# facebookresearch/vggsfm

Hardware: NVIDIA H100
Metric: BA iterations/sec (higher is better)
Workload: dtype f64

## Files before the change

### vggsfm_b200/csrc/ba_schur.cu

```cuda
#include <stddef.h>
#include <algorithm>
#include <vector>
#include "common.cuh"
#include "dev_probes.h"
#include "syrk_work.h"

namespace vgg {

BandDev g_band_dev = {nullptr, nullptr, nullptr, 0};

__device__ __forceinline__ void ar_add(double* local, double* mc, double v) {
  if (mc) asm volatile("multimem.red.relaxed.sys.global.add.f64 [%0], %1;" ::"l"(mc), "d"(v) : "memory");
  else atomicAdd(local, v);
}
__device__ __forceinline__ void ar_put(double* local, double* mc, double v) {
  if (mc) asm volatile("multimem.red.relaxed.sys.global.add.f64 [%0], %1;" ::"l"(mc), "d"(v) : "memory");
  else *local = v;
}

__global__ void jacobi_scale_points_kernel(int N, const double* __restrict__ H_pp, double* __restrict__ sc_p, int enable) {
  const int n = blockIdx.x * blockDim.x + threadIdx.x;
  if (n >= N) return;
  const double* h = H_pp + (size_t)n * 6;
  sc_p[n * 3 + 0] = enable ? 1.0 / (1.0 + sqrt(h[0])) : 1.0;
  sc_p[n * 3 + 1] = enable ? 1.0 / (1.0 + sqrt(h[3])) : 1.0;
  sc_p[n * 3 + 2] = enable ? 1.0 / (1.0 + sqrt(h[5])) : 1.0;
}

__global__ void jacobi_scale_cams_kernel(int D, const double* __restrict__ hdiag, double* __restrict__ sc_c, int enable) {
  const int i = blockIdx.x * blockDim.x + threadIdx.x;
  if (i >= D) return;
  sc_c[i] = enable ? 1.0 / (1.0 + sqrt(hdiag[i])) : 1.0;
}

__global__ void point_prep_kernel(int N, const double* __restrict__ H_pp, const double* __restrict__ g_p,
                                  const double* __restrict__ sc_p, const uint8_t* __restrict__ point_const,
                                  double radius, double min_diag, double max_diag, double* __restrict__ M,
                                  double* __restrict__ q, double* __restrict__ dpp, double* __restrict__ scal) {
  const int n = blockIdx.x * blockDim.x + threadIdx.x;
  if (n >= N) return;
  double* Mo = M + (size_t)n * 9;
  if (point_const && point_const[n]) {
#pragma unroll
    for (int i = 0; i < 9; ++i) Mo[i] = 0.0;
    q[n * 3] = q[n * 3 + 1] = q[n * 3 + 2] = 0.0;
    dpp[n * 3] = dpp[n * 3 + 1] = dpp[n * 3 + 2] = 0.0;
    return;
  }
  const double* h = H_pp + (size_t)n * 6;
  const double s0 = sc_p[n * 3], s1 = sc_p[n * 3 + 1], s2 = sc_p[n * 3 + 2];
  double v00 = h[0] * s0 * s0, v01 = h[1] * s0 * s1, v02 = h[2] * s0 * s2;
  double v11 = h[3] * s1 * s1, v12 = h[4] * s1 * s2, v22 = h[5] * s2 * s2;
  const double d0 = fmin(fmax(v00, min_diag), max_diag);
  const double d1 = fmin(fmax(v11, min_diag), max_diag);
  const double d2 = fmin(fmax(v22, min_diag), max_diag);
  dpp[n * 3] = d0; dpp[n * 3 + 1] = d1; dpp[n * 3 + 2] = d2;
  v00 += d0 / radius; v11 += d1 / radius; v22 += d2 / radius;
  bool bad = !(v00 > 0.0);
  const double l00 = sqrt(v00);
  const double l10 = v01 / l00, l20 = v02 / l00;
  const double t11 = v11 - l10 * l10;
  bad = bad || !(t11 > 0.0);
  const double l11 = sqrt(t11);
  const double l21 = (v12 - l20 * l10) / l11;
  const double t22 = v22 - l20 * l20 - l21 * l21;
  bad = bad || !(t22 > 0.0);
  const double l22 = sqrt(t22);
  if (bad) {
    atomicAdd(&scal[6], 1.0);
#pragma unroll
    for (int i = 0; i < 9; ++i) Mo[i] = 0.0;
    q[n * 3] = q[n * 3 + 1] = q[n * 3 + 2] = 0.0;
    return;
  }
  const double i00 = 1.0 / l00, i11 = 1.0 / l11, i22 = 1.0 / l22;
  const double i10 = -l10 * i00 * i11;
  const double i21 = -l21 * i11 * i22;
  const double i20 = -(l20 * i00 + l21 * i10) * i22;
  const double m00 = s0 * i00, m01 = s0 * i10, m02 = s0 * i20;
  const double m11 = s1 * i11, m12 = s1 * i21;
  const double m22 = s2 * i22;
  Mo[0] = m00; Mo[1] = m01; Mo[2] = m02;
  Mo[3] = 0.0; Mo[4] = m11; Mo[5] = m12;
  Mo[6] = 0.0; Mo[7] = 0.0; Mo[8] = m22;
  const double g0 = g_p[n * 3], g1 = g_p[n * 3 + 1], g2 = g_p[n * 3 + 2];
  q[n * 3 + 0] = m00 * g0;
  q[n * 3 + 1] = m01 * g0 + m11 * g1;
  q[n * 3 + 2] = m02 * g0 + m12 * g1 + m22 * g2;
}

__global__ void assemble_hc_kernel(int S, int dc, int ns, int KR, int Dpad, const double* __restrict__ camrec,
                                   const double* __restrict__ shared_in, double* __restrict__ Sraw,
                                   double* __restrict__ rhs, double* __restrict__ hdiag, double* __restrict__ gvec,
                                   ptrdiff_t mc_off) {
  const int s = blockIdx.x;
  const int tid = threadIdx.x;
#define VGG_PUT(ptr, val) ar_put((ptr), mc_off ? (ptr) + mc_off : nullptr, (val))
  if (s < S) {
    const double* rec = camrec + (size_t)s * KR;
    const int base = s * dc;
    if (tid < dc) {
      VGG_PUT(&gvec[base + tid], rec[tid]);
      VGG_PUT(&rhs[base + tid], -rec[tid]);
    }
    if (tid < dc * dc) {
      const int i = tid / dc, j = tid % dc;
      const int a = i < j ? i : j, b = i < j ? j : i;
      const int idx = dc + a * dc - a * (a - 1) / 2 + (b - a);
      const double val = rec[idx];
      VGG_PUT(&Sraw[(size_t)(base + i) * Dpad + base + j], val);
      if (i == j) VGG_PUT(&hdiag[base + i], val);
    }
    if (tid < 6 * ns) {
      const int i = tid / ns, j = tid % ns;
      const double val = rec[dc + dc * (dc + 1) / 2 + tid];
      VGG_PUT(&Sraw[(size_t)(S * dc + j) * Dpad + base + i], val);
      VGG_PUT(&Sraw[(size_t)(base + i) * Dpad + S * dc + j], val);
    }
  } else if (ns > 0) {
    const int base = S * dc;
    if (tid < ns) {
      VGG_PUT(&gvec[base + tid], shared_in[tid]);
      VGG_PUT(&rhs[base + tid], -shared_in[tid]);
    }
    if (tid < ns * ns) {
      const int i = tid / ns, j = tid % ns;
      const int a = i < j ? i : j, b = i < j ? j : i;
      const double val = shared_in[2 + (a == 0 ? b : 2)];
      VGG_PUT(&Sraw[(size_t)(base + i) * Dpad + base + j], val);
      if (i == j) VGG_PUT(&hdiag[base + i], val);
    }
  }
#undef VGG_PUT
}

constexpr int ZB_NT = 32;
__global__ void __launch_bounds__(128) z_build_kernel(int D, int N, int Dpad, size_t pitch, const double* __restrict__ W,
                                                      const double* __restrict__ M, const double* __restrict__ q,
                                                      double* __restrict__ Zt, double* __restrict__ rhs,
                                                      ptrdiff_t mc_off, const int* __restrict__ rb_range) {
  __shared__ double sm[ZB_NT][12];
  const int row = blockIdx.x * 128 + threadIdx.x;
  const int n0 = blockIdx.y * ZB_NT;
  const int nt = min(ZB_NT, N - n0);
  if (rb_range) {
    const int kb_first = (3 * n0) >> 6, kb_last = (3 * (n0 + nt - 1) + 2) >> 6;
    if (kb_last < rb_range[2 * blockIdx.x] || kb_first >= rb_range[2 * blockIdx.x + 1]) return;
  }
  for (int e = threadIdx.x; e < nt * 12; e += 128) {
    const int t = e / 12, k = e % 12;
    sm[t][k] = k < 9 ? M[(size_t)(n0 + t) * 9 + k] : q[(size_t)(n0 + t) * 3 + (k - 9)];
  }
  __syncthreads();
  if (row >= D) return;
  double zq = 0.0;
  const double* wp = W + ((size_t)n0 * pitch + row) * 3;
#pragma unroll 4
  for (int t = 0; t < nt; ++t, wp += pitch * 3) {
    const double w0 = wp[0], w1 = wp[1], w2 = wp[2];
    const double* m = sm[t];
    const double z0 = w0 * m[0];
    const double z1 = w0 * m[1] + w1 * m[4];
    const double z2 = w0 * m[2] + w1 * m[5] + w2 * m[8];
    double* zo = Zt + (size_t)(3 * (n0 + t)) * Dpad + row;
    zo[0] = z0;
    zo[Dpad] = z1;
    zo[2 * (size_t)Dpad] = z2;
    zq += z0 * m[9] + z1 * m[10] + z2 * m[11];
  }
  if (zq != 0.0) ar_add(&rhs[row], mc_off ? &rhs[row] + mc_off : nullptr, zq);
}

constexpr int SF_BM = 128, SF_BK = 16, SF_LDS = 132, SF_STAGES = 4, SF_MMA_WARPS = 8;
constexpr int SF_THREADS = 128 + SF_MMA_WARPS * 32;
constexpr int SF_STAGE_DOUBLES = 2 * SF_BK * SF_LDS;
constexpr size_t SF_SMEM_BYTES = sizeof(double) * SF_STAGES * SF_STAGE_DOUBLES + sizeof(uint64_t) * 2 * SF_STAGES;

struct SyrkWork {
  int bi, bj, kb0, kb1;
};

__device__ __forceinline__ void dmma_m16n8k16(double (&d)[4], const double (&a)[8], const double (&b)[4]) {
  asm volatile(
      "mma.sync.aligned.m16n8k16.row.col.f64.f64.f64.f64 {%0,%1,%2,%3}, {%4,%5,%6,%7,%8,%9,%10,%11}, {%12,%13,%14,%15}, "
      "{%0,%1,%2,%3};"
      : "+d"(d[0]), "+d"(d[1]), "+d"(d[2]), "+d"(d[3])
      : "d"(a[0]), "d"(a[1]), "d"(a[2]), "d"(a[3]), "d"(a[4]), "d"(a[5]), "d"(a[6]), "d"(a[7]), "d"(b[0]), "d"(b[1]),
        "d"(b[2]), "d"(b[3]));
}

__global__ void __launch_bounds__(SF_THREADS, 1)
    syrk_f64_kernel(const SyrkWork* __restrict__ work, int nwork, int Kpad, int Dpad, const double* __restrict__ Zt,
                    double* __restrict__ Cmat, ptrdiff_t mc_off, int fill_upper, const __grid_constant__ FabricDev fd) {
  extern __shared__ __align__(16) double sf_smem[];
  uint64_t* full = reinterpret_cast<uint64_t*>(sf_smem + SF_STAGES * SF_STAGE_DOUBLES);
  uint64_t* empty = full + SF_STAGES;
  const int warp = threadIdx.x >> 5, lane = threadIdx.x & 31;
  if (threadIdx.x == 0) {
    for (int s = 0; s < SF_STAGES; ++s) {
      mbar_init(&full[s], 1);
      mbar_init(&empty[s], SF_MMA_WARPS);
    }
    mbar_fence_init();
  }
  __syncthreads();

  int stage = 0, phase = 0;
  if (warp < 4) {
    asm volatile("setmaxnreg.dec.sync.aligned.u32 40;");
    if (warp > 0) return;
    const int row = lane & (SF_BK - 1), opnd = lane / SF_BK;
    for (int w = blockIdx.x; w < nwork; w += gridDim.x) {
      const SyrkWork wk = work[w];
      const bool diag = wk.bi == wk.bj;
      const int k1 = min(Kpad, wk.kb1 * 64);
      for (int k = wk.kb0 * 64; k < k1; k += SF_BK) {
        mbar_wait(&empty[stage], phase ^ 1);
        if (lane == 0) mbar_expect_tx(&full[stage], (diag ? 1u : 2u) * SF_BK * SF_BM * (uint32_t)sizeof(double));
        __syncwarp();
        if (opnd == 0 || !diag)
          tma_load_1d(sf_smem + stage * SF_STAGE_DOUBLES + (opnd * SF_BK + row) * SF_LDS,
                      Zt + (size_t)(k + row) * Dpad + (opnd ? wk.bj : wk.bi) * SF_BM, SF_BM * sizeof(double), &full[stage]);
        if (++stage == SF_STAGES) {
          stage = 0;
          phase ^= 1;
        }
      }
    }
    return;
  }

  asm volatile("setmaxnreg.inc.sync.aligned.u32 232;");
  const int wm = (warp - 4) >> 2, wn = warp & 3;
  const int g = lane >> 2, t = lane & 3;
  for (int w = blockIdx.x; w < nwork; w += gridDim.x) {
    const SyrkWork wk = work[w];
    const bool diag = wk.bi == wk.bj;
    const int k1 = min(Kpad, wk.kb1 * 64);
    double acc[4][4][4];
#pragma unroll
    for (int mt = 0; mt < 4; ++mt)
#pragma unroll
      for (int nt = 0; nt < 4; ++nt)
#pragma unroll
        for (int h = 0; h < 4; ++h) acc[mt][nt][h] = 0.0;
    for (int k = wk.kb0 * 64; k < k1; k += SF_BK) {
      mbar_wait(&full[stage], phase);
      const double* as = sf_smem + stage * SF_STAGE_DOUBLES + t * SF_LDS + wm * 64 + g;
      const double* bs = sf_smem + stage * SF_STAGE_DOUBLES + (diag ? 0 : SF_BK * SF_LDS) + t * SF_LDS + wn * 32 + g;
      double b[4][4];
#pragma unroll
      for (int nt = 0; nt < 4; ++nt)
#pragma unroll
        for (int j = 0; j < 4; ++j) b[nt][j] = bs[4 * j * SF_LDS + nt * 8];
#pragma unroll
      for (int mt = 0; mt < 4; ++mt) {
        double a[8];
#pragma unroll
        for (int i = 0; i < 8; ++i) a[i] = as[4 * (i >> 1) * SF_LDS + mt * 16 + 8 * (i & 1)];
#pragma unroll
        for (int nt = 0; nt < 4; ++nt) dmma_m16n8k16(acc[mt][nt], a, b[nt]);
      }
      __syncwarp();
      if (lane == 0) mbar_arrive(&empty[stage]);
      if (++stage == SF_STAGES) {
        stage = 0;
        phase ^= 1;
      }
    }
#pragma unroll
    for (int mt = 0; mt < 4; ++mt)
#pragma unroll
      for (int nt = 0; nt < 4; ++nt)
#pragma unroll
        for (int h = 0; h < 4; ++h) {
          const int r = wk.bi * SF_BM + wm * 64 + mt * 16 + g + 8 * (h >> 1);
          const int col = wk.bj * SF_BM + wn * 32 + nt * 8 + 2 * t + (h & 1);
          syrk_red_upper(Cmat, Dpad, r, col, wk.bj, diag, acc[mt][nt][h], mc_off, fill_upper, fd);
        }
  }
}

__global__ void scale_damp_kernel(int D, int Dpad, double* __restrict__ A, const double* __restrict__ rhs,
                                  const double* __restrict__ hdiag, const double* __restrict__ sc,
                                  const uint8_t* __restrict__ pconst, double radius, double min_diag, double max_diag,
                                  double* __restrict__ bvec, int fill_upper) {
  const int j = blockIdx.x * blockDim.x + threadIdx.x;
  const int i = blockIdx.y;
  if (j >= D || (!fill_upper && j > i)) return;
  const bool ci = pconst[i] != 0, cj = pconst[j] != 0;
  double v;
  if (ci || cj) {
    v = (i == j) ? 1.0 : 0.0;
  } else {
    v = A[(size_t)i * Dpad + j] * sc[i] * sc[j];
    if (i == j) v += fmin(fmax(hdiag[i] * sc[i] * sc[i], min_diag), max_diag) / radius;
  }
  A[(size_t)i * Dpad + j] = v;
  if (i == j) {
    const double b = ci ? 0.0 : rhs[i] * sc[i];
    bvec[i] = b;
    if (fill_upper) A[(size_t)i * Dpad + D] = b;
    else A[(size_t)D * Dpad + i] = b;
    if (i == 0) A[(size_t)D * Dpad + D] = 1e300;
  }
}

__global__ void cam_step_kernel(int D, const double* __restrict__ dcs, size_t dcs_stride, const double* __restrict__ sc,
                                const double* __restrict__ hdiag, const double* __restrict__ gvec,
                                const uint8_t* __restrict__ pconst, double radius, double min_diag, double max_diag,
                                double* __restrict__ d_c, double* __restrict__ scal) {
  const int i = blockIdx.x * blockDim.x + threadIdx.x;
  double a = 0, b = 0, bad = 0;
  if (i < D) {
    const double x = pconst[i] ? 0.0 : dcs[(size_t)i * dcs_stride];
    const double dc = x * sc[i];
    d_c[i] = dc;
    if (!isfinite(x)) bad = 1.0;
    const double dcc = fmin(fmax(hdiag[i] * sc[i] * sc[i], min_diag), max_diag);
    a = pconst[i] ? 0.0 : (x * x * dcc / radius - dc * gvec[i]);
    b = dc * dc;
  }
  a = warp_sum(a); b = warp_sum(b); bad = warp_sum(bad);
  if ((threadIdx.x & 31) == 0) {
    atomicAdd(&scal[0], a);
    atomicAdd(&scal[1], b);
    if (bad > 0) atomicAdd(&scal[7], bad);
  }
}

__global__ void __launch_bounds__(256) backsub_kernel(int D, int N, size_t pitch, const double* __restrict__ W,
                                                      const double* __restrict__ d_c, double* __restrict__ wacc,
                                                      const int* __restrict__ kb_rows, int arrow_row) {
  const int lane = threadIdx.x & 31;
  const int n = blockIdx.x * 8 + (threadIdx.x >> 5);
  if (n >= N) return;
  const double* wp = W + (size_t)n * pitch * 3;
  double w0 = 0, w1 = 0, w2 = 0;
  auto span = [&](int r0, int r1) {
#pragma unroll 4
    for (int r = r0 + lane; r < r1; r += 32) {
      const double d = __ldg(d_c + r);
      w0 = fma(wp[(size_t)r * 3], d, w0);
      w1 = fma(wp[(size_t)r * 3 + 1], d, w1);
      w2 = fma(wp[(size_t)r * 3 + 2], d, w2);
    }
  };
  if (kb_rows) {
    const int ka = (3 * n) >> 6, kb = (3 * n + 2) >> 6;
    const int lo = min(kb_rows[2 * ka], kb_rows[2 * kb]), hi = min(max(kb_rows[2 * ka + 1], kb_rows[2 * kb + 1]), arrow_row);
    if (lo < hi) span(lo, hi);
    span(min(arrow_row, D), D);
  } else {
    span(0, D);
  }
  w0 = warp_sum(w0); w1 = warp_sum(w1); w2 = warp_sum(w2);
  if (lane == 0) {
    wacc[(size_t)n * 3] = w0;
    wacc[(size_t)n * 3 + 1] = w1;
    wacc[(size_t)n * 3 + 2] = w2;
  }
}

__global__ void point_step_kernel(int N, const double* __restrict__ M, const double* __restrict__ g_p,
                                  const double* __restrict__ wacc, const double* __restrict__ sc_p,
                                  const double* __restrict__ dpp, const double* __restrict__ X, double radius,
                                  double* __restrict__ Xc, double* __restrict__ scal) {
  const int n = blockIdx.x * blockDim.x + threadIdx.x;
  double a = 0, b = 0;
  if (n < N) {
    const double* m = M + (size_t)n * 9;
    const double g0 = g_p[n * 3], g1 = g_p[n * 3 + 1], g2 = g_p[n * 3 + 2];
    const double y0 = -(g0 + wacc[n * 3]), y1 = -(g1 + wacc[n * 3 + 1]), y2 = -(g2 + wacc[n * 3 + 2]);
    const double t0 = m[0] * y0;
    const double t1 = m[1] * y0 + m[4] * y1;
    const double t2 = m[2] * y0 + m[5] * y1 + m[8] * y2;
    const double d0 = m[0] * t0 + m[1] * t1 + m[2] * t2;
    const double d1 = m[4] * t1 + m[5] * t2;
    const double d2 = m[8] * t2;
    Xc[n * 3] = X[n * 3] + d0;
    Xc[n * 3 + 1] = X[n * 3 + 1] + d1;
    Xc[n * 3 + 2] = X[n * 3 + 2] + d2;
    const double s0 = sc_p[n * 3], s1 = sc_p[n * 3 + 1], s2 = sc_p[n * 3 + 2];
    const double e0 = d0 / s0, e1 = d1 / s1, e2 = d2 / s2;
    a = (e0 * e0 * dpp[n * 3] + e1 * e1 * dpp[n * 3 + 1] + e2 * e2 * dpp[n * 3 + 2]) / radius -
        (d0 * g0 + d1 * g1 + d2 * g2);
    b = d0 * d0 + d1 * d1 + d2 * d2;
  }
  a = warp_sum(a); b = warp_sum(b);
  if ((threadIdx.x & 31) == 0) {
    atomicAdd(&scal[2], a);
    atomicAdd(&scal[3], b);
  }
}

__global__ void cam_update_kernel(int S, int dc, int ns, int model, const double* __restrict__ d_c,
                                  const double* __restrict__ poses, const double* __restrict__ intr,
                                  double* __restrict__ poses_c, double* __restrict__ intr_c) {
  const int s = blockIdx.x * blockDim.x + threadIdx.x;
  if (s >= S) return;
  const double* d = d_c + (size_t)s * dc;
  const double p0 = 2.0 * d[0], p1 = 2.0 * d[1], p2 = 2.0 * d[2];
  const double th2 = p0 * p0 + p1 * p1 + p2 * p2;
  const double th = sqrt(th2);
  double a, b;
  if (th < 1e-12) {
    a = 1.0 - th2 / 6.0;
    b = 0.5 - th2 / 24.0;
  } else {
    a = sin(th) / th;
    b = (1.0 - cos(th)) / th2;
  }
  double E[9];
  E[0] = 1.0 + b * (-(p1 * p1 + p2 * p2)); E[1] = -a * p2 + b * p0 * p1;           E[2] = a * p1 + b * p0 * p2;
  E[3] = a * p2 + b * p0 * p1;             E[4] = 1.0 + b * (-(p0 * p0 + p2 * p2)); E[5] = -a * p0 + b * p1 * p2;
  E[6] = -a * p1 + b * p0 * p2;            E[7] = a * p0 + b * p1 * p2;            E[8] = 1.0 + b * (-(p0 * p0 + p1 * p1));
  const double* P = poses + (size_t)s * 12;
  double* Q = poses_c + (size_t)s * 12;
#pragma unroll
  for (int i = 0; i < 3; ++i)
#pragma unroll
    for (int j = 0; j < 3; ++j) Q[i * 4 + j] = E[i * 3] * P[j] + E[i * 3 + 1] * P[4 + j] + E[i * 3 + 2] * P[8 + j];
  Q[3] = P[3] + d[3];
  Q[7] = P[7] + d[4];
  Q[11] = P[11] + d[5];
  const int ni = (model == VGG_SIMPLE_PINHOLE) ? 1 : 2;
  double f = intr[s * 4], k = intr[s * 4 + 3];
  if (dc > 6) {
    f += d[6];
    if (ni > 1) k += d[7];
  } else if (ns > 0) {
    const double* dsh = d_c + (size_t)S * dc;
    f += dsh[0];
    if (ni > 1) k += dsh[1];
  }
  intr_c[s * 4] = f;
  intr_c[s * 4 + 1] = intr[s * 4 + 1];
  intr_c[s * 4 + 2] = intr[s * 4 + 2];
  intr_c[s * 4 + 3] = k;
}

__global__ void extract_gvec_kernel(int S, int dc, int ns, int KR, const double* __restrict__ camrec,
                                    const double* __restrict__ shared_in, double* __restrict__ gvec) {
  const int i = blockIdx.x * blockDim.x + threadIdx.x;
  const int D = S * dc + ns;
  if (i >= D) return;
  gvec[i] = (i < S * dc) ? camrec[(size_t)(i / dc) * KR + (i % dc)] : shared_in[i - S * dc];
}

__global__ void gradmax_kernel(int D, int N, const double* __restrict__ gvec, const uint8_t* __restrict__ pconst,
                               const double* __restrict__ g_p, const uint8_t* __restrict__ point_const,
                               double* __restrict__ scal) {
  const int i = blockIdx.x * blockDim.x + threadIdx.x;
  double mc = 0, mp = 0;
  if (i < D && !pconst[i]) mc = fabs(gvec[i]);
  if (i < N * 3 && !(point_const && point_const[i / 3])) mp = fabs(g_p[i]);
  mc = warp_max(mc); mp = warp_max(mp);
  if ((threadIdx.x & 31) == 0) {
    atomicMax(reinterpret_cast<unsigned long long*>(&scal[4]), (unsigned long long)__double_as_longlong(mc));
    atomicMax(reinterpret_cast<unsigned long long*>(&scal[5]), (unsigned long long)__double_as_longlong(mp));
  }
}

int launch_jacobi_scale_points(int N, const double* H_pp, double* sc_p, int enable, cudaStream_t st) {
  jacobi_scale_points_kernel<<<(N + 255) / 256, 256, 0, st>>>(N, H_pp, sc_p, enable);
  VGG_LAUNCH_CHECK();
  return VGG_OK;
}
int launch_jacobi_scale_cams(int D, const double* hdiag, double* sc_c, int enable, cudaStream_t st) {
  jacobi_scale_cams_kernel<<<(D + 255) / 256, 256, 0, st>>>(D, hdiag, sc_c, enable);
  VGG_LAUNCH_CHECK();
  return VGG_OK;
}
int launch_point_prep(int N, const double* H_pp, const double* g_p, const double* sc_p, const uint8_t* point_const,
                      double radius, double min_diag, double max_diag, double* M, double* q, double* dpp,
                      double* scal, cudaStream_t st) {
  point_prep_kernel<<<(N + 127) / 128, 128, 0, st>>>(N, H_pp, g_p, sc_p, point_const, radius, min_diag, max_diag, M, q,
                                                     dpp, scal);
  VGG_LAUNCH_CHECK();
  return VGG_OK;
}
int launch_assemble_hc(int S, int dc, int ns, int KR, int Dpad, const double* camrec, const double* shared_in,
                       double* Sraw, double* rhs, double* hdiag, double* gvec, ptrdiff_t mc_off, cudaStream_t st) {
  assemble_hc_kernel<<<S + (ns > 0 ? 1 : 0), 64, 0, st>>>(S, dc, ns, KR, Dpad, camrec, shared_in, Sraw, rhs, hdiag, gvec,
                                                          mc_off);
  VGG_LAUNCH_CHECK();
  return VGG_OK;
}
int launch_z_transpose(int D, int N, int Dpad, const double* W, const double* M, const double* q, double* Zt,
                       double* rhs, ptrdiff_t mc_off, cudaStream_t st) {
  const size_t pitch = (size_t)(D + (D & 1));
  dim3 grid((D + 127) / 128, (N + ZB_NT - 1) / ZB_NT);
  z_build_kernel<<<grid, 128, 0, st>>>(D, N, Dpad, pitch, W, M, q, Zt, rhs, mc_off, g_band_dev.rb_range);
  VGG_LAUNCH_CHECK();
  return VGG_OK;
}
int g_fill_upper = 0;

FabricDev g_fabric_dev = {0, 0, {nullptr, nullptr, nullptr, nullptr, nullptr, nullptr, nullptr, nullptr}};

extern std::vector<int> g_syrk_kb_ranges;

struct SyrkF64State {
  int dev = -1, Kpad = -1, Dpad = -1, sms = 0, nwork = 0;
  std::vector<int> ranges;
  SyrkWork* work_dev = nullptr;
  size_t work_cap = 0;
};
thread_local SyrkF64State g_sf;

int launch_syrk(int Kpad, int Dpad, const double* Zt, double* Cmat, ptrdiff_t mc_off, cudaStream_t st) {
  VGG_REQUIRE(Dpad % SF_BM == 0 && Kpad % SF_BK == 0, "syrk: Dpad must be a multiple of 128 and Kpad of 16");
  const int nb = Dpad / SF_BM, KB = (Kpad + 63) / 64;
  SyrkF64State& hs = g_sf;
  const std::vector<int> ranges = (int)g_syrk_kb_ranges.size() == 2 * nb ? g_syrk_kb_ranges : std::vector<int>();
  int dev = 0;
  VGG_CUDA_CHECK(cudaGetDevice(&dev));
  if (hs.dev != dev || hs.Kpad != Kpad || hs.Dpad != Dpad || hs.ranges != ranges) {
    VGG_CUDA_CHECK(cudaDeviceGetAttribute(&hs.sms, cudaDevAttrMultiProcessorCount, dev));
    VGG_CUDA_CHECK(cudaFuncSetAttribute(syrk_f64_kernel, cudaFuncAttributeMaxDynamicSharedMemorySize, (int)SF_SMEM_BYTES));
    std::vector<SyrkWork> work;
    build_work_list<SyrkWork>({1}, syrk_tile_jobs(nb, ranges), KB, hs.sms, KB, 1,
                              [](const SyrkTileJob& j, int, int k0, int k1) { return SyrkWork{j.bi, j.bj, k0, k1}; }, &work);
    VGG_CUDA_CHECK(cudaDeviceSynchronize());
    if (hs.dev != dev || work.size() > hs.work_cap) {
      if (hs.work_dev) cudaFree(hs.work_dev);
      hs.work_dev = nullptr;
      hs.work_cap = std::max<size_t>(work.size(), 1);
      VGG_CUDA_CHECK(cudaMalloc(reinterpret_cast<void**>(&hs.work_dev), sizeof(SyrkWork) * hs.work_cap));
    }
    if (!work.empty())
      VGG_CUDA_CHECK(cudaMemcpy(hs.work_dev, work.data(), sizeof(SyrkWork) * work.size(), cudaMemcpyHostToDevice));
    hs.nwork = (int)work.size();
    hs.dev = dev;
    hs.Kpad = Kpad;
    hs.Dpad = Dpad;
    hs.ranges = ranges;
  }
  if (hs.nwork == 0) return VGG_OK;
  syrk_f64_kernel<<<std::min(hs.sms, hs.nwork), SF_THREADS, SF_SMEM_BYTES, st>>>(hs.work_dev, hs.nwork, Kpad, Dpad, Zt, Cmat,
                                                                               mc_off, g_fill_upper, g_fabric_dev);
  VGG_LAUNCH_CHECK();
  return VGG_OK;
}
int launch_scale_damp(int D, int Dpad, double* A, const double* rhs, const double* hdiag, const double* sc,
                      const uint8_t* pconst, double radius, double min_diag, double max_diag, double* bvec,
                      cudaStream_t st) {
  dim3 grid((D + 255) / 256, D);
  scale_damp_kernel<<<grid, 256, 0, st>>>(D, Dpad, A, rhs, hdiag, sc, pconst, radius, min_diag, max_diag, bvec, g_fill_upper);
  VGG_LAUNCH_CHECK();
  return VGG_OK;
}
int launch_cam_step(int D, const double* dcs, size_t dcs_stride, const double* sc, const double* hdiag, const double* gvec,
                    const uint8_t* pconst, double radius, double min_diag, double max_diag, double* d_c, double* scal,
                    cudaStream_t st) {
  cam_step_kernel<<<(D + 255) / 256, 256, 0, st>>>(D, dcs, dcs_stride, sc, hdiag, gvec, pconst, radius, min_diag, max_diag, d_c, scal);
  VGG_LAUNCH_CHECK();
  return VGG_OK;
}
int launch_backsub(int D, int N, const double* W, const double* d_c, double* wacc, cudaStream_t st) {
  const size_t pitch = (size_t)(D + (D & 1));
  backsub_kernel<<<(N + 7) / 8, 256, 0, st>>>(D, N, pitch, W, d_c, wacc, g_band_dev.kb_rows, g_band_dev.arrow_row);
  VGG_LAUNCH_CHECK();
  return VGG_OK;
}
int launch_point_step(int N, const double* M, const double* g_p, const double* wacc, const double* sc_p,
                      const double* dpp, const double* X, double radius, double* Xc, double* scal, cudaStream_t st) {
  point_step_kernel<<<(N + 127) / 128, 128, 0, st>>>(N, M, g_p, wacc, sc_p, dpp, X, radius, Xc, scal);
  VGG_LAUNCH_CHECK();
  return VGG_OK;
}
int launch_cam_update(int S, int dc, int ns, int model, const double* d_c, const double* poses, const double* intr,
                      double* poses_c, double* intr_c, cudaStream_t st) {
  cam_update_kernel<<<(S + 127) / 128, 128, 0, st>>>(S, dc, ns, model, d_c, poses, intr, poses_c, intr_c);
  VGG_LAUNCH_CHECK();
  return VGG_OK;
}
int launch_extract_gvec(int S, int dc, int ns, int KR, const double* camrec, const double* shared_in, double* gvec,
                        cudaStream_t st) {
  const int D = S * dc + ns;
  extract_gvec_kernel<<<(D + 255) / 256, 256, 0, st>>>(S, dc, ns, KR, camrec, shared_in, gvec);
  VGG_LAUNCH_CHECK();
  return VGG_OK;
}
int launch_gradmax(int D, int N, const double* gvec, const uint8_t* pconst, const double* g_p,
                   const uint8_t* point_const, double* scal, cudaStream_t st) {
  const int n = D > N * 3 ? D : N * 3;
  gradmax_kernel<<<(n + 255) / 256, 256, 0, st>>>(D, N, gvec, pconst, g_p, point_const, scal);
  VGG_LAUNCH_CHECK();
  return VGG_OK;
}

}

extern "C" {

int vgg_dev_syrk_f64(int Kpad, int Dpad, const double* Zt, double* Cmat, void* stream) {
  using namespace vgg;
  g_launch_count = 0;
  VGG_REQUIRE(Zt && Cmat && Kpad > 0 && Dpad > 0, "bad argument");
  return launch_syrk(Kpad, Dpad, Zt, Cmat, 0, static_cast<cudaStream_t>(stream));
}

}
```

### vggsfm_b200/csrc/chol.cu

```cuda
#include <stdlib.h>
#include <algorithm>
#include <map>
#include <vector>
#include <tuple>
#include "common.cuh"

namespace vgg {

constexpr int CB = 128;
constexpr int CLD = 132;
constexpr int C_RPC = 16;
constexpr int CT = 64;
constexpr int C_THREADS = 256;

__device__ __forceinline__ void chol_dmma(double& d0, double& d1, double a, double b) {
  asm volatile("mma.sync.aligned.m8n8k4.row.col.f64.f64.f64.f64 {%0,%1}, {%2}, {%3}, {%0,%1};"
               : "+d"(d0), "+d"(d1)
               : "d"(a), "d"(b));
}

__device__ __forceinline__ double fast_rsqrt(double p) {
  double r;
  asm("rsqrt.approx.ftz.f64 %0, %1;" : "=d"(r) : "d"(p));
  const double hp = 0.5 * p;
  r = r * fma(-hp * r, r, 1.5);
  r = r * fma(-hp * r, r, 1.5);
  return r;
}
constexpr double CHOL_PMIN = 2.2250738585072014e-308;

template <int LEAF, bool PROBE>
__device__ __forceinline__ int cta_chol128(double* Ls, double* dinv, int* fail_sm, int tid, int xr,
                                           long long* prof = nullptr) {
  const int lane = tid & 31, warp = tid >> 5;
  __shared__ __align__(16) double Lh[64];
  if (tid == 0) *fail_sm = 0;
  __syncthreads();
  auto tri_row = [](int e) { return (e >= 1) + (e >= 3) + (e >= 6) + (e >= 10) + (e >= 15) + (e >= 21) + (e >= 28); };
  const int pi0 = tri_row(lane), pj0 = lane - pi0 * (pi0 + 1) / 2;
  const int e1 = lane < 4 ? lane + 32 : 35;
  const int pi1 = tri_row(e1), pj1 = e1 - pi1 * (pi1 + 1) / 2;
  long long pacc[6] = {0, 0, 0, 0, 0, 0}, plast = 0;
  const bool ptid = PROBE && (tid == 0 || tid == 32);
  if (ptid) plast = clock64();
#define CHOL_MARK(ph)                         \
  if (ptid) {                                 \
    const long long t_ = clock64();           \
    pacc[ph] += t_ - plast;                   \
    plast = t_;                               \
  }
  auto leaf1 = [&](int c0) {
    double a[8];
    const int r = c0 + (lane & 7);
#pragma unroll
    for (int c = 0; c < 8; c += 2) {
      const double2 v = *reinterpret_cast<const double2*>(Ls + r * CLD + c0 + c);
      a[c] = v.x;
      a[c + 1] = v.y;
    }
    int fail = 0;
    double mydinv = 1.0;
#pragma unroll
    for (int j = 0; j < 8; j += 2) {
      const double A = __shfl_sync(0xffffffffu, a[j], j);
      const double B = __shfl_sync(0xffffffffu, a[j], j + 1);
      const double C = __shfl_sync(0xffffffffu, a[j + 1], j + 1);
      const double AC = A * C;
      const double det = fma(-B, B, AC);
      double ia = fast_rsqrt(A);
      double ib = (A * ia) * fast_rsqrt(det);
      double l10 = B * ia;
      const bool good = A >= CHOL_PMIN && det >= CHOL_PMIN && AC < 1e280 && AC > 1e-280;
      if (!good) {
        if (!(A >= CHOL_PMIN)) {
          if (fail == 0) fail = c0 + j + 1;
          ia = 1.0;
          l10 = B;
        }
        const double p1 = fma(-l10, l10, C);
        if (!(p1 >= CHOL_PMIN)) {
          if (fail == 0) fail = c0 + j + 2;
          ib = 1.0;
        } else {
          ib = rsqrt(p1);
        }
      }
      const double x0 = a[j] * ia;
      const double x1 = fma(-x0, l10, a[j + 1]) * ib;
      a[j] = x0;
      a[j + 1] = x1;
      if (lane == j) {
        dinv[c0 + j] = ia;
        dinv[c0 + j + 1] = ib;
        mydinv = ia;
      }
      if (lane == j + 1) mydinv = ib;
#pragma unroll
      for (int c = j + 2; c < 8; ++c) {
        const double l0 = __shfl_sync(0xffffffffu, x0, c);
        const double l1 = __shfl_sync(0xffffffffu, x1, c);
        if (lane >= c) a[c] = fma(-x1, l1, fma(-x0, l0, a[c]));
      }
    }
    if (lane < 8) {
#pragma unroll
      for (int c = 0; c < 8; ++c) Ls[r * CLD + c0 + c] = (c <= lane) ? a[c] : 0.0;
#pragma unroll
      for (int c = 0; c < 8; ++c) Lh[lane * 8 + c] = (c < lane) ? a[c] * mydinv : 0.0;
    }
    if (lane == 0 && fail && *fail_sm == 0) *fail_sm = fail;
  };
  auto leaf0 = [&](int c0) {
    double a[8];
    const int r = c0 + (lane & 7);
#pragma unroll
    for (int c = 0; c < 8; c += 2) {
      const double2 v = *reinterpret_cast<const double2*>(Ls + r * CLD + c0 + c);
      a[c] = v.x;
      a[c + 1] = v.y;
    }
    int fail = 0;
    double mydinv = 1.0;
#pragma unroll
    for (int j = 0; j < 8; ++j) {
      const double pj = __shfl_sync(0xffffffffu, a[j], j);
      double inv = fast_rsqrt(pj);
      if (!(pj >= CHOL_PMIN)) {
        if (fail == 0) fail = c0 + j + 1;
        inv = 1.0;
      }
      a[j] = a[j] * inv;
      if (lane == j) {
        dinv[c0 + j] = inv;
        mydinv = inv;
      }
#pragma unroll
      for (int c = j + 1; c < 8; ++c) {
        const double lc = __shfl_sync(0xffffffffu, a[j], c);
        if (lane >= c) a[c] = fma(-a[j], lc, a[c]);
      }
    }
    if (lane < 8) {
#pragma unroll
      for (int c = 0; c < 8; ++c) Ls[r * CLD + c0 + c] = (c <= lane) ? a[c] : 0.0;
#pragma unroll
      for (int c = 0; c < 8; ++c) Lh[lane * 8 + c] = (c < lane) ? a[c] * mydinv : 0.0;
    }
    if (lane == 0 && fail && *fail_sm == 0) *fail_sm = fail;
  };
  auto leaf = [&](int c0) {
    if constexpr (LEAF == 0) leaf0(c0);
    else leaf1(c0);
  };
  auto row_update = [&](int r, int c0, int jb, int js, int jend) {
    double li[8];
#pragma unroll
    for (int k = 0; k < 8; k += 2) {
      const double2 v = *reinterpret_cast<const double2*>(Ls + r * CLD + c0 + k);
      li[k] = v.x;
      li[k + 1] = v.y;
    }
    int j = jb;
    for (; j + js <= jend; j += 2 * js) {
      const double* l0 = Ls + j * CLD + c0;
      const double* l1 = Ls + (j + js) * CLD + c0;
      double s0 = Ls[r * CLD + j], s1 = Ls[r * CLD + j + js];
#pragma unroll
      for (int k = 0; k < 8; k += 2) {
        const double2 u = *reinterpret_cast<const double2*>(l0 + k);
        const double2 w = *reinterpret_cast<const double2*>(l1 + k);
        s0 = fma(-li[k], u.x, s0);
        s1 = fma(-li[k], w.x, s1);
        s0 = fma(-li[k + 1], u.y, s0);
        s1 = fma(-li[k + 1], w.y, s1);
      }
      Ls[r * CLD + j] = s0;
      Ls[r * CLD + j + js] = s1;
    }
    if (j <= jend) {
      const double* l0 = Ls + j * CLD + c0;
      double s0 = Ls[r * CLD + j];
#pragma unroll
      for (int k = 0; k < 8; k += 2) {
        const double2 u = *reinterpret_cast<const double2*>(l0 + k);
        s0 = fma(-li[k], u.x, s0);
        s0 = fma(-li[k + 1], u.y, s0);
      }
      Ls[r * CLD + j] = s0;
    }
  };
  if (warp == 0) leaf(0);
  __syncthreads();
  CHOL_MARK(0)
  for (int sp = 0; sp < CB / 32; ++sp) {
    const int c32 = sp * 32;
    for (int mp = 0; mp < 4; ++mp) {
      const int c0 = c32 + mp * 8;
      {
        const int r = c0 + 8 + tid;
        if (r < CB + xr) {
          double x[8];
#pragma unroll
          for (int c = 0; c < 8; c += 2) {
            const double2 v = *reinterpret_cast<const double2*>(Ls + r * CLD + c0 + c);
            x[c] = v.x;
            x[c + 1] = v.y;
          }
#pragma unroll
          for (int m = 0; m < 8; ++m) x[m] *= dinv[c0 + m];
#pragma unroll
          for (int m = 1; m < 8; ++m) {
#pragma unroll
            for (int k = 0; k < m; ++k) x[m] = fma(-x[k], Lh[m * 8 + k], x[m]);
          }
#pragma unroll
          for (int c = 0; c < 8; c += 2) *reinterpret_cast<double2*>(Ls + r * CLD + c0 + c) = make_double2(x[c], x[c + 1]);
        }
      }
      __syncthreads();
      CHOL_MARK(1)
      if (mp < 3) {
        const int n0 = c0 + 8;
        if (warp == 0) {
          {
            const double* ri = Ls + (n0 + pi0) * CLD + c0;
            const double* rj = Ls + (n0 + pj0) * CLD + c0;
            const double* ri1 = Ls + (n0 + pi1) * CLD + c0;
            const double* rj1 = Ls + (n0 + pj1) * CLD + c0;
            double s0 = Ls[(n0 + pi0) * CLD + n0 + pj0], s1 = 0.0;
            double u0 = Ls[(n0 + pi1) * CLD + n0 + pj1], u1 = 0.0;
#pragma unroll
            for (int k = 0; k < 8; k += 4) {
              const double2 a0 = *reinterpret_cast<const double2*>(ri + k), a1 = *reinterpret_cast<const double2*>(ri + k + 2);
              const double2 b0 = *reinterpret_cast<const double2*>(rj + k), b1 = *reinterpret_cast<const double2*>(rj + k + 2);
              const double2 c0v = *reinterpret_cast<const double2*>(ri1 + k), c1v = *reinterpret_cast<const double2*>(ri1 + k + 2);
              const double2 d0 = *reinterpret_cast<const double2*>(rj1 + k), d1 = *reinterpret_cast<const double2*>(rj1 + k + 2);
              s0 = fma(-a0.x, b0.x, s0);
              s1 = fma(-a0.y, b0.y, s1);
              u0 = fma(-c0v.x, d0.x, u0);
              u1 = fma(-c0v.y, d0.y, u1);
              s0 = fma(-a1.x, b1.x, s0);
              s1 = fma(-a1.y, b1.y, s1);
              u0 = fma(-c1v.x, d1.x, u0);
              u1 = fma(-c1v.y, d1.y, u1);
            }
            Ls[(n0 + pi0) * CLD + n0 + pj0] = s0 + s1;
            if (lane < 4) Ls[(n0 + pi1) * CLD + n0 + pj1] = u0 + u1;
          }
          __syncwarp();
          leaf(n0);
        } else {
          const int t = tid - 32;
          for (int rr = t >> 1; n0 + rr < CB + xr; rr += 112) {
            const int r = n0 + rr, half = t & 1;
            const int jend = min(r, c32 + 31);
            if (r < n0 + 8) continue;
            row_update(r, c0, n0 + half, 2, jend);
          }
        }
        CHOL_MARK(2)
        __syncthreads();
        CHOL_MARK(3)
      }
    }
    const int t0 = c32 + 32;
    const int nrb = (CB - t0) / 32;
    if (nrb > 0) {
      const int ntile = nrb * (nrb + 1);
      const int nxt = xr ? (CB - t0) / 16 : 0;
      const int g = lane >> 2, q = lane & 3;
      bool leaf_pending = warp == 0;
      for (int t = warp == 0 ? 0 : warp; t < ntile + nxt; t += (warp == 0 ? ntile + nxt : C_THREADS / 32 - 1)) {
        int R0, C0, nrow8 = 4;
        if (t < ntile) {
          int rb = 0, cb = t;
          while (cb >= 2 * rb + 2) { cb -= 2 * rb + 2; ++rb; }
          R0 = t0 + rb * 32;
          C0 = t0 + cb * 16;
        } else {
          R0 = CB;
          C0 = t0 + (t - ntile) * 16;
          nrow8 = 2;
        }
        double c[4][2][2];
#pragma unroll
        for (int i = 0; i < 4; ++i)
#pragma unroll
          for (int j = 0; j < 2; ++j) c[i][j][0] = c[i][j][1] = 0.0;
        const double* arow = Ls + (R0 + g) * CLD + c32 + q;
        const double* brow = Ls + (C0 + g) * CLD + c32 + q;
#pragma unroll
        for (int k4 = 0; k4 < 8; ++k4) {
          double a[4], b[2];
#pragma unroll
          for (int i = 0; i < 4; ++i) a[i] = (i < nrow8) ? arow[i * 8 * CLD + k4 * 4] : 0.0;
#pragma unroll
          for (int j = 0; j < 2; ++j) b[j] = brow[j * 8 * CLD + k4 * 4];
#pragma unroll
          for (int i = 0; i < 4; ++i) {
            if (i < nrow8) {
#pragma unroll
              for (int j = 0; j < 2; ++j) chol_dmma(c[i][j][0], c[i][j][1], a[i], b[j]);
            }
          }
        }
#pragma unroll
        for (int i = 0; i < 4; ++i) {
          if (i >= nrow8) continue;
          const int r = R0 + i * 8 + g;
#pragma unroll
          for (int j = 0; j < 2; ++j) {
            const int col = C0 + j * 8 + 2 * q;
            if (col > r) continue;
            double* pp = Ls + r * CLD + col;
            if (col + 1 <= r) {
              double2 v = *reinterpret_cast<double2*>(pp);
              v.x -= c[i][j][0];
              v.y -= c[i][j][1];
              *reinterpret_cast<double2*>(pp) = v;
            } else {
              *pp -= c[i][j][0];
            }
          }
        }
        if (leaf_pending) {
          __syncwarp();
          leaf(t0);
          leaf_pending = false;
        }
      }
      CHOL_MARK(4)
      __syncthreads();
      CHOL_MARK(5)
    }
  }
#undef CHOL_MARK
  if (ptid) {
#pragma unroll
    for (int i = 0; i < 6; ++i) prof[(tid == 32 ? 6 : 0) + i] = pacc[i];
  }
  return *fail_sm;
}

template <int LEAF>
__global__ void __launch_bounds__(C_THREADS, 1) chol128_probe_kernel(const double* __restrict__ A, double* __restrict__ L,
                                                                      long long* __restrict__ prof, int reps, int xr) {
  extern __shared__ __align__(16) double cp_smem[];
  __shared__ double dinv[CB];
  __shared__ int fail_sm;
  const int tid = threadIdx.x;
  long long total = 0;
  for (int rep = 0; rep < reps; ++rep) {
    for (int e = tid; e < CB * CB; e += C_THREADS) cp_smem[(e >> 7) * CLD + (e & 127)] = A[e];
    for (int e = tid; e < xr * CB; e += C_THREADS)
      cp_smem[(CB + (e >> 7)) * CLD + (e & 127)] = A[(CB - xr + (e >> 7)) * CB + (e & 127)];
    __syncthreads();
    const long long t0 = clock64();
    cta_chol128<LEAF, true>(cp_smem, dinv, &fail_sm, tid, xr, prof);
    __syncthreads();
    total = clock64() - t0;
  }
  if (tid == 0) prof[12] = total;
  for (int e = tid; e < CB * CB; e += C_THREADS) L[e] = ((e & 127) <= (e >> 7)) ? cp_smem[(e >> 7) * CLD + (e & 127)] : 0.0;
}

constexpr int CHOL_SPIN_LIMIT = 1 << 22;
constexpr int CHOL_INFO_STALLED = 0x7fffffff;

template <int LEAF>
__global__ void __launch_bounds__(C_THREADS, 1) chol_panel_kernel(int n, int lda, int k0, double* __restrict__ A,
                                                                   double* __restrict__ Ldiag ,
                                                                   int* __restrict__ info, int* __restrict__ flags,
                                                                   int fuse, int band_end, int arrow_lo) {
  extern __shared__ __align__(16) double cp_smem[];
  double* Ls = cp_smem;
  double* Ts = cp_smem + CB * CLD;
  __shared__ double dinv[CB];
  __shared__ int fail_sm;
  const int tid = threadIdx.x, lane = tid & 31, warp = tid >> 5;
  const int nb = min(CB, n - k0);
  const bool solver = blockIdx.x > 0;
  const int chunks1r = (max(0, min(band_end, n) - (k0 + CB)) + C_RPC - 1) / C_RPC;
  const int cidx = (int)blockIdx.x - 1;
  const int r0 = cidx < chunks1r ? k0 + CB + cidx * C_RPC : arrow_lo + (cidx - chunks1r) * C_RPC;
  for (int e = tid; e < CB * (CB / 2); e += C_THREADS) {
    const int i = e >> 6, j = (e & 63) * 2;
    if (i < nb) {
      cp_async16(Ls + i * CLD + j, A + (size_t)(k0 + i) * lda + k0 + j);
    } else {
      *reinterpret_cast<double2*>(Ls + i * CLD + j) = make_double2(j == i ? 1.0 : 0.0, j + 1 == i ? 1.0 : 0.0);
    }
  }
  for (int e = tid; e < C_RPC * (CB / 2); e += C_THREADS) {
    const int r = e >> 6, j = (e & 63) * 2;
    if (solver && r0 + r < n) cp_async16(Ts + r * CLD + j, A + (size_t)(r0 + r) * lda + k0 + j);
    else *reinterpret_cast<double2*>(Ts + r * CLD + j) = make_double2(0.0, 0.0);
  }
  cp_async_commit();
  cp_async_wait<0>();
  __syncthreads();
  const int fail = cta_chol128<LEAF, false>(Ls, dinv, &fail_sm, tid, C_RPC);
  if (fail && blockIdx.x == 0 && tid == 0) atomicCAS(info, 0, k0 + fail);
  if (!solver) {
    const bool alone = gridDim.x == 1;
    double* dst = Ldiag + (size_t)(k0 / CB) * CB * CB;
    for (int e = tid; e < CB * CB; e += C_THREADS) {
      const int i = e >> 7, j = e & 127;
      if (i < nb && j < nb) {
        if (j > i) A[(size_t)(k0 + i) * lda + k0 + j] = Ls[j * CLD + i];
        else if (alone) A[(size_t)(k0 + i) * lda + k0 + j] = Ls[i * CLD + j];
        else dst[e] = Ls[i * CLD + j];
      }
    }
    if (k0 > 0) {
      const double* src = Ldiag + (size_t)(k0 / CB - 1) * CB * CB;
      double* blk = A + (size_t)(k0 - CB) * lda + (k0 - CB);
      for (int e0 = tid; e0 < CB * CB; e0 += 8 * C_THREADS) {
        double v[8];
#pragma unroll
        for (int u = 0; u < 8; ++u) {
          const int e = e0 + u * C_THREADS;
          v[u] = ((e & 127) <= (e >> 7)) ? __ldcg(src + e) : 0.0;
        }
#pragma unroll
        for (int u = 0; u < 8; ++u) {
          const int e = e0 + u * C_THREADS;
          const int i = e >> 7, j = e & 127;
          if (j <= i) blk[(size_t)i * lda + j] = v[u];
        }
      }
    }
    return;
  }
  for (int e = tid; e < C_RPC * CB; e += C_THREADS) {
    const int r = e >> 7, c = e & 127;
    if (r0 + r < n && c < nb) A[(size_t)(r0 + r) * lda + k0 + c] = Ts[r * CLD + c];
  }
  for (int e = tid; e < C_RPC * CB; e += C_THREADS) {
    const int c = e >> 4, r = e & 15;
    if (r0 + r < n && c < nb) A[(size_t)(k0 + c) * lda + r0 + r] = Ts[r * CLD + c];
  }
  if (!fuse) return;

  const int t0 = k0 + CB;
  const bool p_active = band_end > t0 || arrow_lo == t0;
  const int nprod = p_active ? min(CB / C_RPC, (int)gridDim.x - 1) : 0;
  if (nprod == 0) return;
  int* flag = flags + k0 / CB;
  __threadfence();
  __syncthreads();
  if (tid == 0) {
    if ((int)blockIdx.x <= nprod) atomicAdd(flag, 1);
    int spins = 0, seen;
    do {
      asm volatile("ld.acquire.gpu.global.s32 %0, [%1];" : "=r"(seen) : "l"(flag) : "memory");
    } while (seen < nprod && ++spins < CHOL_SPIN_LIMIT);
    if (seen < nprod) atomicCAS(info, 0, CHOL_INFO_STALLED);
  }
  __syncthreads();
#pragma unroll
  for (int half = 0; half < 2; ++half) {
    for (int e = tid; e < CB * 16; e += C_THREADS) {
      const int row = e >> 4, ch = (e & 15) * 4 + half * 64;
      double* dst = Ls + row * CLD + ch;
      if (t0 + row < n) {
        const double* src = A + (size_t)(t0 + row) * lda + k0 + ch;
        cp_async16(dst, src);
        cp_async16(dst + 2, src + 2);
      } else {
        *reinterpret_cast<double2*>(dst) = make_double2(0.0, 0.0);
        *reinterpret_cast<double2*>(dst + 2) = make_double2(0.0, 0.0);
      }
    }
    cp_async_commit();
  }
  {
    const int g = lane >> 2, q = lane & 3;
    double c[2][2][2];
#pragma unroll
    for (int i = 0; i < 2; ++i)
#pragma unroll
      for (int j = 0; j < 2; ++j) c[i][j][0] = c[i][j][1] = 0.0;
    const double* arow = Ts + g * CLD + q;
    const double* brow = Ls + (warp * 16 + g) * CLD + q;
#pragma unroll
    for (int half = 0; half < 2; ++half) {
      if (half == 0) cp_async_wait<1>();
      else cp_async_wait<0>();
      __syncthreads();
#pragma unroll 4
      for (int k4 = half * 16; k4 < half * 16 + 16; ++k4) {
        double a[2], b[2];
#pragma unroll
        for (int i = 0; i < 2; ++i) a[i] = arow[i * 8 * CLD + k4 * 4];
#pragma unroll
        for (int j = 0; j < 2; ++j) b[j] = brow[j * 8 * CLD + k4 * 4];
#pragma unroll
        for (int i = 0; i < 2; ++i)
#pragma unroll
          for (int j = 0; j < 2; ++j) chol_dmma(c[i][j][0], c[i][j][1], a[i], b[j]);
      }
    }
#pragma unroll
    for (int i = 0; i < 2; ++i) {
      const int r = r0 + i * 8 + g;
      if (r >= n) continue;
#pragma unroll
      for (int j = 0; j < 2; ++j) {
        const int col = t0 + warp * 16 + j * 8 + 2 * q;
        double* p = A + (size_t)r * lda + col;
        if (col <= r) atomicAdd(p, -c[i][j][0]);
        if (col + 1 <= r) atomicAdd(p + 1, -c[i][j][1]);
      }
    }
  }
}

constexpr int CUD = 68;
template <int TM>
__global__ void __launch_bounds__(C_THREADS, 2) chol_update_kernel(int n, int lda, int k0, int t0, int mode,
                                                                    double* __restrict__ A, int band_end, int arrow_lo,
                                                                    int all_red, int ntiles) {
  constexpr int WN = TM == 64 ? 4 : 8;
  constexpr int NJ = 64 / WN / 8;
  extern __shared__ __align__(16) double cu_smem[];
  double* As = cu_smem;
  double* Bs = cu_smem + TM * CUD;
  for (int tile_t = blockIdx.x; tile_t < ntiles; tile_t += gridDim.x) {
  int bi, bj;
  {
    int t = tile_t;
    if (TM == 32) {
      const int T = (n - t0 + 31) / 32;
      if (t < T) { bi = t; bj = 0; }
      else { bi = t - T + 2; bj = 1; }
    } else if (mode == 4) {
      const int T = (max(0, min(band_end, n) - t0) + 63) / 64 + (band_end >= n ? 0 : (n - arrow_lo + 63) / 64);
      if (t < T - 2) { bi = 2 + t; bj = 2; }
      else { bi = 3 + (t - (T - 2)); bj = 3; }
    } else {
      bi = (int)((sqrtf(8.0f * (float)t + 1.0f) - 1.0f) * 0.5f);
      while ((bi + 1) * (bi + 2) / 2 <= t) ++bi;
      while (bi * (bi + 1) / 2 > t) --bi;
      bj = t - bi * (bi + 1) / 2;
      const int skip = mode == 5 ? 4 : (mode >= 2 ? 2 : 0);
      bi += skip;
      bj += skip;
    }
  }
  const bool diag = TM == 64 && bi == bj;
  const int tid = threadIdx.x, lane = tid & 31, warp = tid >> 5;
  const int T1v = band_end >= n ? (1 << 30) : (band_end - t0) / 64;
  auto vrow = [&](int v) { return v < T1v ? t0 + v * 64 : arrow_lo + (v - T1v) * 64; };
  const int ri = TM == 64 ? vrow(bi) : t0 + bi * TM, rj = TM == 64 ? vrow(bj) : t0 + bj * 64;
  const double* bs = diag ? As : Bs;
  const int wm = warp / WN, wn = warp % WN;
  const int g = lane >> 2, q = lane & 3;
  double c[4][NJ][2];
#pragma unroll
  for (int i = 0; i < 4; ++i)
#pragma unroll
    for (int j = 0; j < NJ; ++j) c[i][j][0] = c[i][j][1] = 0.0;
  const double* arow = As + (wm * 32 + g) * CUD + q;
  const double* brow = bs + (wn * (8 * NJ) + g) * CUD + q;
#pragma unroll 1
  for (int half = 0; half < 2; ++half) {
    if (half) __syncthreads();
    for (int e = tid; e < (TM + 64) * 16; e += C_THREADS) {
      const int row = e >> 4, ch = (e & 15) * 4;
      const bool isA = row < TM;
      if (!isA && diag) continue;
      const int grow = isA ? ri + row : rj + (row - TM);
      double* dst = (isA ? As + row * CUD : Bs + (row - TM) * CUD) + ch;
      if (grow < n) {
        const double* src = A + (size_t)grow * lda + k0 + half * 64 + ch;
        cp_async16(dst, src);
        cp_async16(dst + 2, src + 2);
      } else {
        *reinterpret_cast<double2*>(dst) = make_double2(0.0, 0.0);
        *reinterpret_cast<double2*>(dst + 2) = make_double2(0.0, 0.0);
      }
    }
    cp_async_commit();
    cp_async_wait<0>();
    __syncthreads();
#pragma unroll 4
    for (int k4 = 0; k4 < 16; ++k4) {
      double a[4], b[NJ];
#pragma unroll
      for (int i = 0; i < 4; ++i) a[i] = arow[i * 8 * CUD + k4 * 4];
#pragma unroll
      for (int j = 0; j < NJ; ++j) b[j] = brow[j * 8 * CUD + k4 * 4];
#pragma unroll
      for (int i = 0; i < 4; ++i)
#pragma unroll
        for (int j = 0; j < NJ; ++j) chol_dmma(c[i][j][0], c[i][j][1], a[i], b[j]);
    }
  }
#pragma unroll
  for (int i = 0; i < 4; ++i) {
    const int r = ri + wm * 32 + i * 8 + g;
    if (r >= n) continue;
#pragma unroll
    for (int j = 0; j < NJ; ++j) {
      const int col = rj + wn * (8 * NJ) + j * 8 + 2 * q;
      if (col > r) continue;
      double* p = A + (size_t)r * lda + col;
      if (TM == 64 && (all_red || (mode == 3 && bj < 4) || mode == 4 || (mode == 5 && bj < 6))) {
        atomicAdd(p, -c[i][j][0]);
        if (col + 1 <= r) atomicAdd(p + 1, -c[i][j][1]);
      } else if (col + 1 <= r) {
        double2 v = *reinterpret_cast<double2*>(p);
        v.x -= c[i][j][0];
        v.y -= c[i][j][1];
        *reinterpret_cast<double2*>(p) = v;
      } else {
        *p -= c[i][j][0];
      }
    }
  }
  __syncthreads();
  }
}


size_t chol_workspace_doubles(int n) {
  const int nblk = (n + CB - 1) / CB;
  return (size_t)nblk * CB * CB + (size_t)(nblk + 1) / 2 + 1;
}

namespace {

struct CholStreams {
  cudaStream_t side = nullptr, side_lo = nullptr, side_mid = nullptr, cap = nullptr;
  cudaEvent_t ev_col = nullptr, ev_panel = nullptr, ev_upd[2] = {nullptr, nullptr}, ev_bulk[3] = {nullptr, nullptr, nullptr};
  bool ready = false;
};

int chol_streams(CholStreams** out) {
  static thread_local CholStreams s;
  if (!s.ready) {
    int lo = 0, hi = 0;
    VGG_CUDA_CHECK(cudaDeviceGetStreamPriorityRange(&lo, &hi));
    VGG_CUDA_CHECK(cudaStreamCreateWithPriority(&s.side, cudaStreamNonBlocking, hi));
    VGG_CUDA_CHECK(cudaStreamCreateWithPriority(&s.side_lo, cudaStreamNonBlocking, lo));
    VGG_CUDA_CHECK(cudaStreamCreateWithPriority(&s.side_mid, cudaStreamNonBlocking, (lo + hi) / 2));
    VGG_CUDA_CHECK(cudaStreamCreateWithPriority(&s.cap, cudaStreamNonBlocking, hi));
    VGG_CUDA_CHECK(cudaEventCreateWithFlags(&s.ev_col, cudaEventDisableTiming));
    VGG_CUDA_CHECK(cudaEventCreateWithFlags(&s.ev_panel, cudaEventDisableTiming));
    VGG_CUDA_CHECK(cudaEventCreateWithFlags(&s.ev_upd[0], cudaEventDisableTiming));
    VGG_CUDA_CHECK(cudaEventCreateWithFlags(&s.ev_upd[1], cudaEventDisableTiming));
    for (int i = 0; i < 3; ++i) VGG_CUDA_CHECK(cudaEventCreateWithFlags(&s.ev_bulk[i], cudaEventDisableTiming));
    s.ready = true;
  }
  *out = &s;
  return VGG_OK;
}

int chol_leaf() {
  static const int v = [] { const char* e = getenv("VGG_CHOL_LEAF"); return (e && e[0] == '0') ? 0 : 1; }();
  return v;
}

int chol_set_attrs() {
  static bool done = false;
  if (done) return VGG_OK;
  VGG_CUDA_CHECK(cudaFuncSetAttribute(chol_panel_kernel<0>, cudaFuncAttributeMaxDynamicSharedMemorySize,
                                      (int)(sizeof(double) * (CB + C_RPC) * CLD)));
  VGG_CUDA_CHECK(cudaFuncSetAttribute(chol_panel_kernel<1>, cudaFuncAttributeMaxDynamicSharedMemorySize,
                                      (int)(sizeof(double) * (CB + C_RPC) * CLD)));
  VGG_CUDA_CHECK(cudaFuncSetAttribute(chol_update_kernel<64>, cudaFuncAttributeMaxDynamicSharedMemorySize,
                                      (int)(sizeof(double) * 2 * CT * CUD)));
  VGG_CUDA_CHECK(cudaFuncSetAttribute(chol_update_kernel<32>, cudaFuncAttributeMaxDynamicSharedMemorySize,
                                      (int)(sizeof(double) * (32 + CT) * CUD)));
  done = true;
  return VGG_OK;
}

}

std::vector<int> g_chol_band_end;
int g_chol_arrow_blk = 0;

namespace {

bool chol_fuse() {
  static const bool v = [] { const char* e = getenv("VGG_CHOL_FUSE"); return !(e && e[0] == '0'); }();
  return v;
}

int chol_enqueue(int n, int lda, double* A, double* Ldiag, int* info, int* flags, cudaStream_t st, CholStreams* cs,
                 bool lookahead) {
  const int nblk = (n + CB - 1) / CB;
  const size_t smem_p = sizeof(double) * (CB + C_RPC) * CLD;
  const size_t smem_u = sizeof(double) * 2 * CT * CUD;
  const bool fuse = lookahead && chol_fuse();
  static const int persist_ctas = [] {
    const char* e = getenv("VGG_CHOL_PERSIST");
    if (!(e && e[0] == '1')) return 0;
    int dev = 0, sms = 132;
    cudaGetDevice(&dev);
    cudaDeviceGetAttribute(&sms, cudaDevAttrMultiProcessorCount, dev);
    return sms;
  }();
  auto upd_grid = [&](int tiles) { return persist_ctas > 0 ? std::min(tiles, persist_ctas) : tiles; };
  static const bool split = [] { const char* e = getenv("VGG_CHOL_SPLIT"); return !(e && e[0] == '0'); }();
  const bool banded = fuse && split && (int)g_chol_band_end.size() >= nblk && g_chol_arrow_blk > 0;
  auto band_rows = [&](int b, int* band_end, int* arrow_lo) {
    if (!banded) {
      *band_end = *arrow_lo = n;
      return;
    }
    *band_end = std::min(n, g_chol_band_end[b] * CB);
    *arrow_lo = std::min(n, std::max(g_chol_arrow_blk * CB, *band_end));
    if (*band_end >= n || *arrow_lo <= *band_end) *band_end = *arrow_lo = n;
  };
  auto panel = [&](int b, cudaStream_t s2) -> int {
    const int k0 = b * CB;
    int band_end, arrow_lo;
    band_rows(b, &band_end, &arrow_lo);
    const int below1 = std::max(0, std::min(band_end, n) - (k0 + CB));
    const int below2 = band_end >= n ? 0 : n - arrow_lo;
    const int chunks = (below1 + C_RPC - 1) / C_RPC + (below2 + C_RPC - 1) / C_RPC;
    if (chol_leaf() == 1)
      chol_panel_kernel<1><<<1 + chunks, C_THREADS, smem_p, s2>>>(n, lda, k0, A, Ldiag, info, flags, fuse ? 1 : 0, band_end, arrow_lo);
    else
      chol_panel_kernel<0><<<1 + chunks, C_THREADS, smem_p, s2>>>(n, lda, k0, A, Ldiag, info, flags, fuse ? 1 : 0, band_end, arrow_lo);
    VGG_LAUNCH_CHECK();
    return VGG_OK;
  };
  int rc;
  if ((rc = panel(0, st))) return rc;
  if (fuse) {
    static const bool skip_bulk = getenv("VGG_CHOL_TIMING_SKIP_BULK") != nullptr;
    bool have_u1[2] = {false, false}, have_u2[3] = {false, false, false};
    for (int b = 0; b + 1 < nblk; ++b) {
      const int k0 = b * CB, t0 = k0 + CB;
      int band_end, arrow_lo;
      band_rows(b, &band_end, &arrow_lo);
      const int T = (std::max(0, std::min(band_end, n) - t0) + CT - 1) / CT + (band_end >= n ? 0 : (n - arrow_lo + CT - 1) / CT);
      const int all_red = band_end >= n ? 0 : 1;
      const int n_u1 = T > 2 ? (T - 2) + (T > 3 ? T - 3 : 0) : 0;
      const int n_u2 = T > 4 ? (T - 4) * (T - 3) / 2 : 0;
      const int n_rest = T > 2 ? (T - 2) * (T - 1) / 2 : 0;
      have_u1[b & 1] = false;
      have_u2[b % 3] = false;
      if (n_rest > 0 && !skip_bulk) {
        VGG_CUDA_CHECK(cudaEventRecord(cs->ev_col, st));
        if (split) {
          VGG_CUDA_CHECK(cudaStreamWaitEvent(cs->side_mid, cs->ev_col, 0));
          if (b >= 2 && have_u2[(b - 2) % 3]) VGG_CUDA_CHECK(cudaStreamWaitEvent(cs->side_mid, cs->ev_bulk[(b - 2) % 3], 0));
          chol_update_kernel<64><<<upd_grid(n_u1), C_THREADS, smem_u, cs->side_mid>>>(n, lda, k0, t0, 4, A, band_end, arrow_lo, all_red, n_u1);
          VGG_LAUNCH_CHECK();
          VGG_CUDA_CHECK(cudaEventRecord(cs->ev_upd[b & 1], cs->side_mid));
          have_u1[b & 1] = true;
          if (n_u2 > 0) {
            VGG_CUDA_CHECK(cudaStreamWaitEvent(cs->side_lo, cs->ev_col, 0));
            chol_update_kernel<64><<<upd_grid(n_u2), C_THREADS, smem_u, cs->side_lo>>>(n, lda, k0, t0, 5, A, band_end, arrow_lo, all_red, n_u2);
            VGG_LAUNCH_CHECK();
            VGG_CUDA_CHECK(cudaEventRecord(cs->ev_bulk[b % 3], cs->side_lo));
            have_u2[b % 3] = true;
          }
        } else {
          VGG_CUDA_CHECK(cudaStreamWaitEvent(cs->side_lo, cs->ev_col, 0));
          chol_update_kernel<64><<<upd_grid(n_rest), C_THREADS, smem_u, cs->side_lo>>>(n, lda, k0, t0, 3, A, n, n, 0, n_rest);
          VGG_LAUNCH_CHECK();
          VGG_CUDA_CHECK(cudaEventRecord(cs->ev_upd[b & 1], cs->side_lo));
          have_u1[b & 1] = true;
        }
      }
      if (b >= 1 && have_u1[(b - 1) & 1]) VGG_CUDA_CHECK(cudaStreamWaitEvent(st, cs->ev_upd[(b - 1) & 1], 0));
      if (b >= 2 && have_u2[(b - 2) % 3]) VGG_CUDA_CHECK(cudaStreamWaitEvent(st, cs->ev_bulk[(b - 2) % 3], 0));
      if ((rc = panel(b + 1, st))) return rc;
    }
    for (int i = 0; i < 2; ++i)
      if (have_u1[i]) VGG_CUDA_CHECK(cudaStreamWaitEvent(st, cs->ev_upd[i], 0));
    for (int i = 0; i < 3; ++i)
      if (have_u2[i]) VGG_CUDA_CHECK(cudaStreamWaitEvent(st, cs->ev_bulk[i], 0));
    return VGG_OK;
  }
  for (int b = 0; b + 1 < nblk; ++b) {
    const int k0 = b * CB, t0 = k0 + CB;
    const int T = (n - t0 + CT - 1) / CT;
    const int T32 = (n - t0 + 31) / 32;
    const int n_col = T32 + (T32 > 2 ? T32 - 2 : 0);
    const int n_rest = T > 2 ? (T - 2) * (T - 1) / 2 : 0;
    if (!lookahead) {
      chol_update_kernel<64><<<upd_grid(T * (T + 1) / 2), C_THREADS, smem_u, st>>>(n, lda, k0, t0, 0, A, n, n, 0, T * (T + 1) / 2);
      VGG_LAUNCH_CHECK();
      if ((rc = panel(b + 1, st))) return rc;
      continue;
    }
    chol_update_kernel<32><<<n_col, C_THREADS, sizeof(double) * (32 + CT) * CUD, st>>>(n, lda, k0, t0, 1, A, n, n, 0, n_col);
    VGG_LAUNCH_CHECK();
    VGG_CUDA_CHECK(cudaEventRecord(cs->ev_col, st));
    VGG_CUDA_CHECK(cudaStreamWaitEvent(cs->side, cs->ev_col, 0));
    if ((rc = panel(b + 1, cs->side))) return rc;
    VGG_CUDA_CHECK(cudaEventRecord(cs->ev_panel, cs->side));
    if (n_rest > 0) {
      chol_update_kernel<64><<<upd_grid(n_rest), C_THREADS, smem_u, st>>>(n, lda, k0, t0, 2, A, n, n, 0, n_rest);
      VGG_LAUNCH_CHECK();
    }
    VGG_CUDA_CHECK(cudaStreamWaitEvent(st, cs->ev_panel, 0));
  }
  return VGG_OK;
}

}

int chol_lower_inplace(int n, int lda, double* A, double* Ldiag, int* info, cudaStream_t st) {
  VGG_REQUIRE((lda % 2) == 0, "lda must be even");
  int rc;
  if ((rc = chol_set_attrs())) return rc;
  VGG_CUDA_CHECK(cudaMemsetAsync(info, 0, sizeof(int), st));
  const int nblk0 = (n + CB - 1) / CB;
  int* flags = reinterpret_cast<int*>(Ldiag + (size_t)nblk0 * CB * CB);
  VGG_CUDA_CHECK(cudaMemsetAsync(flags, 0, sizeof(int) * (size_t)nblk0, st));
  static const bool lookahead = [] { const char* e = getenv("VGG_CHOL_LOOKAHEAD"); return !(e && e[0] == '0'); }();
  static const bool use_graph = [] { const char* e = getenv("VGG_CHOL_GRAPH"); return !(e && e[0] == '0'); }();
  const int nblk = (n + CB - 1) / CB;
  CholStreams* cs = nullptr;
  if ((rc = chol_streams(&cs))) return rc;
  if (nblk < 3 || !use_graph) return chol_enqueue(n, lda, A, Ldiag, info, flags, st, cs, lookahead && nblk >= 3);
  typedef std::tuple<double*, int, int, int*, double*, bool, unsigned long long> Key;
  static thread_local std::map<Key, cudaGraphExec_t> cache;
  unsigned long long band_hash = (unsigned long long)g_chol_arrow_blk;
  for (int v : g_chol_band_end) band_hash = band_hash * 1000003ull + (unsigned long long)(v + 1);
  const Key key(A, n, lda, info, Ldiag, lookahead, band_hash);
  auto it = cache.find(key);
  if (it == cache.end()) {
    const long long launches_before = g_launch_count;
    cudaGraph_t graph = nullptr;
    VGG_CUDA_CHECK(cudaStreamBeginCapture(cs->cap, cudaStreamCaptureModeThreadLocal));
    rc = chol_enqueue(n, lda, A, Ldiag, info, flags, cs->cap, cs, lookahead);
    const cudaError_t ce = cudaStreamEndCapture(cs->cap, &graph);
    g_launch_count = launches_before;
    if (rc) {
      if (graph) cudaGraphDestroy(graph);
      return rc;
    }
    VGG_CUDA_CHECK(ce);
    cudaGraphExec_t exec = nullptr;
    VGG_CUDA_CHECK(cudaGraphInstantiate(&exec, graph, 0));
    cudaGraphDestroy(graph);
    if (cache.size() > 8) {
      for (auto& kv : cache) cudaGraphExecDestroy(kv.second);
      cache.clear();
    }
    it = cache.emplace(key, exec).first;
  }
  VGG_CUDA_CHECK(cudaGraphLaunch(it->second, st));
  g_launch_count += 1 + 3 * (nblk - 1);
  return VGG_OK;
}

}

extern "C" int vgg_dev_chol128_probe(int leaf, int reps, const double* A_host, double* L_host, long long* prof13_host) {
  using namespace vgg;
  VGG_REQUIRE(A_host && L_host && prof13_host && reps > 0, "chol128 probe: bad arguments");
  double *dA = nullptr, *dL = nullptr;
  long long* dP = nullptr;
  VGG_CUDA_CHECK(cudaMalloc(&dA, sizeof(double) * CB * CB));
  VGG_CUDA_CHECK(cudaMalloc(&dL, sizeof(double) * CB * CB));
  VGG_CUDA_CHECK(cudaMalloc(&dP, sizeof(long long) * 13));
  VGG_CUDA_CHECK(cudaMemcpy(dA, A_host, sizeof(double) * CB * CB, cudaMemcpyHostToDevice));
  VGG_CUDA_CHECK(cudaMemset(dP, 0, sizeof(long long) * 13));
  const int smem = (int)(sizeof(double) * (CB + C_RPC) * CLD);
  if (leaf == 1) {
    VGG_CUDA_CHECK(cudaFuncSetAttribute(chol128_probe_kernel<1>, cudaFuncAttributeMaxDynamicSharedMemorySize, smem));
    chol128_probe_kernel<1><<<1, C_THREADS, smem>>>(dA, dL, dP, reps, C_RPC);
  } else {
    VGG_CUDA_CHECK(cudaFuncSetAttribute(chol128_probe_kernel<0>, cudaFuncAttributeMaxDynamicSharedMemorySize, smem));
    chol128_probe_kernel<0><<<1, C_THREADS, smem>>>(dA, dL, dP, reps, C_RPC);
  }
  VGG_LAUNCH_CHECK();
  VGG_CUDA_CHECK(cudaDeviceSynchronize());
  VGG_CUDA_CHECK(cudaMemcpy(L_host, dL, sizeof(double) * CB * CB, cudaMemcpyDeviceToHost));
  VGG_CUDA_CHECK(cudaMemcpy(prof13_host, dP, sizeof(long long) * 13, cudaMemcpyDeviceToHost));
  cudaFree(dA);
  cudaFree(dL);
  cudaFree(dP);
  return VGG_OK;
}

extern "C" int vgg_dev_set_chol_band(const int* end_blk_host, int count, int arrow_blk) {
  using namespace vgg;
  g_chol_band_end.assign(end_blk_host, end_blk_host + (count > 0 ? count : 0));
  g_chol_arrow_blk = count > 0 ? arrow_blk : 0;
  return VGG_OK;
}
```

### vggsfm_b200/csrc/common.cuh

```cuda
#pragma once
#include <cuda_runtime.h>
#include <stdint.h>
#include <stdio.h>
#include <stdarg.h>
#include "../../include/vggsfm_b200.h"

namespace vgg {

void set_error(const char* fmt, ...);
extern thread_local long long g_launch_count;

#define VGG_CUDA_CHECK(expr)                                                              \
  do {                                                                                    \
    cudaError_t _e = (expr);                                                              \
    if (_e != cudaSuccess) {                                                              \
      vgg::set_error("%s:%d: %s -> %s", __FILE__, __LINE__, #expr, cudaGetErrorString(_e)); \
      return VGG_ECUDA;                                                                   \
    }                                                                                     \
  } while (0)

#define VGG_LAUNCH_CHECK()                 \
  do {                                     \
    vgg::g_launch_count++;                 \
    VGG_CUDA_CHECK(cudaGetLastError());    \
  } while (0)

#define VGG_REQUIRE(cond, msg)                                   \
  do {                                                           \
    if (!(cond)) {                                               \
      vgg::set_error("%s:%d: %s", __FILE__, __LINE__, msg);      \
      return VGG_EINVAL;                                         \
    }                                                            \
  } while (0)

__host__ __device__ constexpr inline size_t align_up(size_t x, size_t a) { return (x + a - 1) / a * a; }

struct Carver {
  char* base;
  size_t off = 0, cap;
  Carver(void* p, size_t c) : base(static_cast<char*>(p)), cap(c) {}
  template <typename T>
  T* take(size_t n) {
    off = align_up(off, 256);
    T* r = reinterpret_cast<T*>(base + off);
    off += n * sizeof(T);
    return r;
  }
  bool ok() const { return base == nullptr || off <= cap; }
};

struct BandDev {
  const int* rb_range;
  const int* kb_rows;
  const int* fg_tracks;
  int arrow_row;
};

struct FabricDev {
  int world, rank;
  double* peer[8];
};

#ifdef __CUDACC__
__device__ __forceinline__ uint32_t smem_u32(const void* p) {
  return static_cast<uint32_t>(__cvta_generic_to_shared(p));
}
__device__ __forceinline__ void mbar_init(uint64_t* bar, uint32_t count) {
  asm volatile("mbarrier.init.shared::cta.b64 [%0], %1;" ::"r"(smem_u32(bar)), "r"(count));
}
__device__ __forceinline__ void mbar_fence_init() {
  asm volatile("fence.mbarrier_init.release.cluster;" ::: "memory");
}
__device__ __forceinline__ void mbar_expect_tx(uint64_t* bar, uint32_t bytes) {
  asm volatile("mbarrier.arrive.expect_tx.shared::cta.b64 _, [%0], %1;" ::"r"(smem_u32(bar)), "r"(bytes)
               : "memory");
}
__device__ __forceinline__ void mbar_arrive(uint64_t* bar) {
  asm volatile("mbarrier.arrive.shared::cta.b64 _, [%0];" ::"r"(smem_u32(bar)) : "memory");
}
__device__ __forceinline__ void mbar_wait(uint64_t* bar, uint32_t parity) {
  asm volatile(
      "{\n"
      ".reg .pred p;\n"
      "WAIT_LOOP:\n"
      "mbarrier.try_wait.parity.shared::cta.b64 p, [%0], %1;\n"
      "@p bra DONE;\n"
      "bra WAIT_LOOP;\n"
      "DONE:\n"
      "}\n" ::"r"(smem_u32(bar)),
      "r"(parity)
      : "memory");
}
__device__ __forceinline__ void tma_load_1d(void* smem_dst, const void* gmem_src, uint32_t bytes, uint64_t* bar) {
  asm volatile(
      "cp.async.bulk.shared::cluster.global.mbarrier::complete_tx::bytes [%0], [%1], %2, [%3];" ::"r"(
          smem_u32(smem_dst)),
      "l"(gmem_src), "r"(bytes), "r"(smem_u32(bar))
      : "memory");
}
__device__ __forceinline__ void tma_store_1d(void* gmem_dst, const void* smem_src, uint32_t bytes) {
  asm volatile("cp.async.bulk.global.shared::cta.bulk_group [%0], [%1], %2;" ::"l"(gmem_dst),
               "r"(smem_u32(smem_src)), "r"(bytes)
               : "memory");
}
__device__ __forceinline__ void tma_store_commit() { asm volatile("cp.async.bulk.commit_group;" ::: "memory"); }
template <int N>
__device__ __forceinline__ void tma_store_wait_read() {
  asm volatile("cp.async.bulk.wait_group.read %0;" ::"n"(N) : "memory");
}
template <int N>
__device__ __forceinline__ void tma_store_wait_all() {
  asm volatile("cp.async.bulk.wait_group %0;" ::"n"(N) : "memory");
}
__device__ __forceinline__ void fence_proxy_async() { asm volatile("fence.proxy.async.shared::cta;" ::: "memory"); }

__device__ __forceinline__ uint64_t wgmma_desc_sw64(uint32_t saddr) {
  return (uint64_t)((saddr >> 4) & 0x3FFF) | (1ull << 16) | ((uint64_t)(512 >> 4) << 32) | (2ull << 62);
}
__device__ __forceinline__ void wgmma_fence() { asm volatile("wgmma.fence.sync.aligned;" ::: "memory"); }
__device__ __forceinline__ void wgmma_commit() { asm volatile("wgmma.commit_group.sync.aligned;" ::: "memory"); }
__device__ __forceinline__ void wgmma_wait_all() { asm volatile("wgmma.wait_group.sync.aligned 0;" ::: "memory"); }

__device__ __forceinline__ void cp_async16(void* smem_dst, const void* gmem_src) {
  asm volatile("cp.async.cg.shared.global [%0], [%1], 16;" ::"r"(smem_u32(smem_dst)), "l"(gmem_src) : "memory");
}
__device__ __forceinline__ void cp_async4(void* smem_dst, const void* gmem_src) {
  asm volatile("cp.async.ca.shared.global [%0], [%1], 4;" ::"r"(smem_u32(smem_dst)), "l"(gmem_src) : "memory");
}
__device__ __forceinline__ void cp_async_commit() { asm volatile("cp.async.commit_group;" ::: "memory"); }
template <int N>
__device__ __forceinline__ void cp_async_wait() {
  asm volatile("cp.async.wait_group %0;" ::"n"(N) : "memory");
}

template <int KP>
__device__ __forceinline__ double warp_reduce_scatter(double (&v)[KP], int lane) {
#pragma unroll
  for (int off = KP / 2; off >= 1; off >>= 1) {
    const bool up = (lane & off) != 0;
#pragma unroll
    for (int i = 0; i < off; ++i) {
      const double mine = up ? v[i + off] : v[i];
      const double send = up ? v[i] : v[i + off];
      v[i] = mine + __shfl_xor_sync(0xffffffffu, send, off);
    }
  }
  double r = v[0];
#pragma unroll
  for (int off = KP; off < 32; off <<= 1) r += __shfl_xor_sync(0xffffffffu, r, off);
  return r;
}

__device__ __forceinline__ double warp_sum(double r) {
#pragma unroll
  for (int off = 16; off >= 1; off >>= 1) r += __shfl_xor_sync(0xffffffffu, r, off);
  return r;
}
__device__ __forceinline__ double warp_max(double r) {
#pragma unroll
  for (int off = 16; off >= 1; off >>= 1) r = fmax(r, __shfl_xor_sync(0xffffffffu, r, off));
  return r;
}

__device__ __forceinline__ void syrk_red_upper(double* Cmat, int Dpad, int r, int col, int bj, bool diag, double v,
                                               ptrdiff_t mc_off, int fill_upper, const FabricDev& fd) {
  if (v == 0.0) return;
  if (!diag || col >= r) {
    const size_t off = (size_t)col * Dpad + r;
    if (fd.world > 1) {
      asm volatile("red.relaxed.sys.global.add.f64 [%0], %1;" ::"l"(fd.peer[bj % fd.world] + off), "d"(-v) : "memory");
    } else if (mc_off) {
      asm volatile("multimem.red.relaxed.sys.global.add.f64 [%0], %1;" ::"l"(Cmat + off + mc_off), "d"(-v) : "memory");
    } else {
      atomicAdd(Cmat + off, -v);
    }
  }
  if (fill_upper && (!diag || col > r)) atomicAdd(&Cmat[(size_t)r * Dpad + col], -v);
}
#endif

}
```

Baseline: 285.3.

## Switch Cholesky kernels to m16n8k16 DMMA with adaptive panel row chunks

Replaces the m8n8k4 f64 MMA in the Cholesky panel, trailing-tile and update kernels with the larger m16n8k16 DMMA shape, which is moved into a shared header. Panel solver blocks now take a runtime row-chunk size (xr, up to 32) chosen per panel instead of a fixed 16, and panel shared memory is sized to match. The host schedule is simplified: the TM=32 column-update variant, the persistent grid-stride loop and the non-split lookahead path are removed in favour of the banded side-stream schedule. The larger MMA shape cuts instruction count per flop, at the cost of more register pressure and a different work split that may change occupancy and overlap.

```diff
diff --git a/vggsfm_b200/csrc/ba_schur.cu b/vggsfm_b200/csrc/ba_schur.cu
--- a/vggsfm_b200/csrc/ba_schur.cu
+++ b/vggsfm_b200/csrc/ba_schur.cu
@@ -179,15 +179,6 @@
 struct SyrkWork {
   int bi, bj, kb0, kb1;
 };
-
-__device__ __forceinline__ void dmma_m16n8k16(double (&d)[4], const double (&a)[8], const double (&b)[4]) {
-  asm volatile(
-      "mma.sync.aligned.m16n8k16.row.col.f64.f64.f64.f64 {%0,%1,%2,%3}, {%4,%5,%6,%7,%8,%9,%10,%11}, {%12,%13,%14,%15}, "
-      "{%0,%1,%2,%3};"
-      : "+d"(d[0]), "+d"(d[1]), "+d"(d[2]), "+d"(d[3])
-      : "d"(a[0]), "d"(a[1]), "d"(a[2]), "d"(a[3]), "d"(a[4]), "d"(a[5]), "d"(a[6]), "d"(a[7]), "d"(b[0]), "d"(b[1]),
-        "d"(b[2]), "d"(b[3]));
-}
 
 __global__ void __launch_bounds__(SF_THREADS, 1)
     syrk_f64_kernel(const SyrkWork* __restrict__ work, int nwork, int Kpad, int Dpad, const double* __restrict__ Zt,
diff --git a/vggsfm_b200/csrc/chol.cu b/vggsfm_b200/csrc/chol.cu
--- a/vggsfm_b200/csrc/chol.cu
+++ b/vggsfm_b200/csrc/chol.cu
@@ -10,14 +10,9 @@
 constexpr int CB = 128;
 constexpr int CLD = 132;
 constexpr int C_RPC = 16;
+constexpr int C_RPC_MAX = 32;
 constexpr int CT = 64;
 constexpr int C_THREADS = 256;
-
-__device__ __forceinline__ void chol_dmma(double& d0, double& d1, double a, double b) {
-  asm volatile("mma.sync.aligned.m8n8k4.row.col.f64.f64.f64.f64 {%0,%1}, {%2}, {%3}, {%0,%1};"
-               : "+d"(d0), "+d"(d1)
-               : "d"(a), "d"(b));
-}
 
 __device__ __forceinline__ double fast_rsqrt(double p) {
   double r;
@@ -268,10 +263,11 @@
     if (nrb > 0) {
       const int ntile = nrb * (nrb + 1);
       const int nxt = xr ? (CB - t0) / 16 : 0;
+      const int rend = CB + xr;
       const int g = lane >> 2, q = lane & 3;
       bool leaf_pending = warp == 0;
       for (int t = warp == 0 ? 0 : warp; t < ntile + nxt; t += (warp == 0 ? ntile + nxt : C_THREADS / 32 - 1)) {
-        int R0, C0, nrow8 = 4;
+        int R0, C0, nrow16 = 2;
         if (t < ntile) {
           int rb = 0, cb = t;
           while (cb >= 2 * rb + 2) { cb -= 2 * rb + 2; ++rb; }
@@ -280,46 +276,53 @@
         } else {
           R0 = CB;
           C0 = t0 + (t - ntile) * 16;
-          nrow8 = 2;
-        }
-        double c[4][2][2];
-#pragma unroll
-        for (int i = 0; i < 4; ++i)
-#pragma unroll
-          for (int j = 0; j < 2; ++j) c[i][j][0] = c[i][j][1] = 0.0;
-        const double* arow = Ls + (R0 + g) * CLD + c32 + q;
-        const double* brow = Ls + (C0 + g) * CLD + c32 + q;
-#pragma unroll
-        for (int k4 = 0; k4 < 8; ++k4) {
-          double a[4], b[2];
-#pragma unroll
-          for (int i = 0; i < 4; ++i) a[i] = (i < nrow8) ? arow[i * 8 * CLD + k4 * 4] : 0.0;
-#pragma unroll
-          for (int j = 0; j < 2; ++j) b[j] = brow[j * 8 * CLD + k4 * 4];
-#pragma unroll
-          for (int i = 0; i < 4; ++i) {
-            if (i < nrow8) {
-#pragma unroll
-              for (int j = 0; j < 2; ++j) chol_dmma(c[i][j][0], c[i][j][1], a[i], b[j]);
+          nrow16 = (xr + 15) / 16;
+        }
+        double c[2][2][4];
+#pragma unroll
+        for (int i = 0; i < 2; ++i)
+#pragma unroll
+          for (int j = 0; j < 2; ++j) c[i][j][0] = c[i][j][1] = c[i][j][2] = c[i][j][3] = 0.0;
+#pragma unroll
+        for (int kk = c32; kk < c32 + 32; kk += 16) {
+          double a[2][8], b[2][4];
+#pragma unroll
+          for (int j = 0; j < 2; ++j)
+#pragma unroll
+            for (int e = 0; e < 4; ++e) b[j][e] = Ls[(C0 + j * 8 + g) * CLD + kk + q + 4 * e];
+#pragma unroll
+          for (int i = 0; i < 2; ++i) {
+            if (i < nrow16) {
+#pragma unroll
+              for (int e = 0; e < 8; ++e) {
+                const int r = R0 + i * 16 + g + 8 * (e & 1);
+                a[i][e] = r < rend ? Ls[r * CLD + kk + q + 4 * (e >> 1)] : 0.0;
+              }
+#pragma unroll
+              for (int j = 0; j < 2; ++j) dmma_m16n8k16(c[i][j], a[i], b[j]);
             }
           }
         }
 #pragma unroll
-        for (int i = 0; i < 4; ++i) {
-          if (i >= nrow8) continue;
-          const int r = R0 + i * 8 + g;
-#pragma unroll
-          for (int j = 0; j < 2; ++j) {
-            const int col = C0 + j * 8 + 2 * q;
-            if (col > r) continue;
-            double* pp = Ls + r * CLD + col;
-            if (col + 1 <= r) {
-              double2 v = *reinterpret_cast<double2*>(pp);
-              v.x -= c[i][j][0];
-              v.y -= c[i][j][1];
-              *reinterpret_cast<double2*>(pp) = v;
-            } else {
-              *pp -= c[i][j][0];
+        for (int i = 0; i < 2; ++i) {
+          if (i >= nrow16) continue;
+#pragma unroll
+          for (int h = 0; h < 2; ++h) {
+            const int r = R0 + i * 16 + g + 8 * h;
+            if (r >= rend) continue;
+#pragma unroll
+            for (int j = 0; j < 2; ++j) {
+              const int col = C0 + j * 8 + 2 * q;
+              if (col > r) continue;
+              double* pp = Ls + r * CLD + col;
+              if (col + 1 <= r) {
+                double2 v = *reinterpret_cast<double2*>(pp);
+                v.x -= c[i][j][2 * h];
+                v.y -= c[i][j][2 * h + 1];
+                *reinterpret_cast<double2*>(pp) = v;
+              } else {
+                *pp -= c[i][j][2 * h];
+              }
             }
           }
         }
@@ -371,7 +374,7 @@
 __global__ void __launch_bounds__(C_THREADS, 1) chol_panel_kernel(int n, int lda, int k0, double* __restrict__ A,
                                                                    double* __restrict__ Ldiag ,
                                                                    int* __restrict__ info, int* __restrict__ flags,
-                                                                   int fuse, int band_end, int arrow_lo) {
+                                                                   int fuse, int band_end, int arrow_lo, int xr) {
   extern __shared__ __align__(16) double cp_smem[];
   double* Ls = cp_smem;
   double* Ts = cp_smem + CB * CLD;
@@ -380,9 +383,11 @@
   const int tid = threadIdx.x, lane = tid & 31, warp = tid >> 5;
   const int nb = min(CB, n - k0);
   const bool solver = blockIdx.x > 0;
-  const int chunks1r = (max(0, min(band_end, n) - (k0 + CB)) + C_RPC - 1) / C_RPC;
+  const int band_hi = min(band_end, n);
+  const int chunks1r = (max(0, band_hi - (k0 + CB)) + xr - 1) / xr;
   const int cidx = (int)blockIdx.x - 1;
-  const int r0 = cidx < chunks1r ? k0 + CB + cidx * C_RPC : arrow_lo + (cidx - chunks1r) * C_RPC;
+  const int r0 = cidx < chunks1r ? k0 + CB + cidx * xr : arrow_lo + (cidx - chunks1r) * xr;
+  const int nrows = solver ? min(xr, (cidx < chunks1r ? band_hi : n) - r0) : 0;
   for (int e = tid; e < CB * (CB / 2); e += C_THREADS) {
     const int i = e >> 6, j = (e & 63) * 2;
     if (i < nb) {
@@ -391,15 +396,15 @@
       *reinterpret_cast<double2*>(Ls + i * CLD + j) = make_double2(j == i ? 1.0 : 0.0, j + 1 == i ? 1.0 : 0.0);
     }
   }
-  for (int e = tid; e < C_RPC * (CB / 2); e += C_THREADS) {
+  for (int e = tid; e < xr * (CB / 2); e += C_THREADS) {
     const int r = e >> 6, j = (e & 63) * 2;
-    if (solver && r0 + r < n) cp_async16(Ts + r * CLD + j, A + (size_t)(r0 + r) * lda + k0 + j);
+    if (r < nrows) cp_async16(Ts + r * CLD + j, A + (size_t)(r0 + r) * lda + k0 + j);
     else *reinterpret_cast<double2*>(Ts + r * CLD + j) = make_double2(0.0, 0.0);
   }
   cp_async_commit();
   cp_async_wait<0>();
   __syncthreads();
-  const int fail = cta_chol128<LEAF, false>(Ls, dinv, &fail_sm, tid, C_RPC);
+  const int fail = cta_chol128<LEAF, false>(Ls, dinv, &fail_sm, tid, xr);
   if (fail && blockIdx.x == 0 && tid == 0) atomicCAS(info, 0, k0 + fail);
   if (!solver) {
     const bool alone = gridDim.x == 1;
@@ -432,19 +437,19 @@
     }
     return;
   }
-  for (int e = tid; e < C_RPC * CB; e += C_THREADS) {
+  for (int e = tid; e < nrows * CB; e += C_THREADS) {
     const int r = e >> 7, c = e & 127;
-    if (r0 + r < n && c < nb) A[(size_t)(r0 + r) * lda + k0 + c] = Ts[r * CLD + c];
-  }
-  for (int e = tid; e < C_RPC * CB; e += C_THREADS) {
-    const int c = e >> 4, r = e & 15;
-    if (r0 + r < n && c < nb) A[(size_t)(k0 + c) * lda + r0 + r] = Ts[r * CLD + c];
+    if (c < nb) A[(size_t)(r0 + r) * lda + k0 + c] = Ts[r * CLD + c];
+  }
+  for (int e = tid; e < nrows * CB; e += C_THREADS) {
+    const int c = e / nrows, r = e - c * nrows;
+    if (c < nb) A[(size_t)(k0 + c) * lda + r0 + r] = Ts[r * CLD + c];
   }
   if (!fuse) return;
 
   const int t0 = k0 + CB;
   const bool p_active = band_end > t0 || arrow_lo == t0;
-  const int nprod = p_active ? min(CB / C_RPC, (int)gridDim.x - 1) : 0;
+  const int nprod = p_active ? min((CB + xr - 1) / xr, (int)gridDim.x - 1) : 0;
   if (nprod == 0) return;
   int* flag = flags + k0 / CB;
   __threadfence();
@@ -476,65 +481,69 @@
   }
   {
     const int g = lane >> 2, q = lane & 3;
-    double c[2][2][2];
+    const int nrow16 = (xr + 15) / 16;
+    double c[2][2][4];
 #pragma unroll
     for (int i = 0; i < 2; ++i)
 #pragma unroll
-      for (int j = 0; j < 2; ++j) c[i][j][0] = c[i][j][1] = 0.0;
-    const double* arow = Ts + g * CLD + q;
-    const double* brow = Ls + (warp * 16 + g) * CLD + q;
+      for (int j = 0; j < 2; ++j) c[i][j][0] = c[i][j][1] = c[i][j][2] = c[i][j][3] = 0.0;
 #pragma unroll
     for (int half = 0; half < 2; ++half) {
       if (half == 0) cp_async_wait<1>();
       else cp_async_wait<0>();
       __syncthreads();
-#pragma unroll 4
-      for (int k4 = half * 16; k4 < half * 16 + 16; ++k4) {
-        double a[2], b[2];
-#pragma unroll
-        for (int i = 0; i < 2; ++i) a[i] = arow[i * 8 * CLD + k4 * 4];
-#pragma unroll
-        for (int j = 0; j < 2; ++j) b[j] = brow[j * 8 * CLD + k4 * 4];
-#pragma unroll
-        for (int i = 0; i < 2; ++i)
-#pragma unroll
-          for (int j = 0; j < 2; ++j) chol_dmma(c[i][j][0], c[i][j][1], a[i], b[j]);
+#pragma unroll 2
+      for (int kk = half * 64; kk < half * 64 + 64; kk += 16) {
+        double a[2][8], b[2][4];
+#pragma unroll
+        for (int j = 0; j < 2; ++j)
+#pragma unroll
+          for (int e = 0; e < 4; ++e) b[j][e] = Ls[(warp * 16 + j * 8 + g) * CLD + kk + q + 4 * e];
+#pragma unroll
+        for (int i = 0; i < 2; ++i) {
+          if (i < nrow16) {
+#pragma unroll
+            for (int e = 0; e < 8; ++e) {
+              const int r = i * 16 + g + 8 * (e & 1);
+              a[i][e] = r < xr ? Ts[r * CLD + kk + q + 4 * (e >> 1)] : 0.0;
+            }
+#pragma unroll
+            for (int j = 0; j < 2; ++j) dmma_m16n8k16(c[i][j], a[i], b[j]);
+          }
+        }
       }
     }
 #pragma unroll
     for (int i = 0; i < 2; ++i) {
-      const int r = r0 + i * 8 + g;
-      if (r >= n) continue;
-#pragma unroll
-      for (int j = 0; j < 2; ++j) {
-        const int col = t0 + warp * 16 + j * 8 + 2 * q;
-        double* p = A + (size_t)r * lda + col;
-        if (col <= r) atomicAdd(p, -c[i][j][0]);
-        if (col + 1 <= r) atomicAdd(p + 1, -c[i][j][1]);
+#pragma unroll
+      for (int h = 0; h < 2; ++h) {
+        const int rr = i * 16 + g + 8 * h;
+        if (i >= nrow16 || rr >= nrows) continue;
+        const int r = r0 + rr;
+#pragma unroll
+        for (int j = 0; j < 2; ++j) {
+          const int col = t0 + warp * 16 + j * 8 + 2 * q;
+          double* p = A + (size_t)r * lda + col;
+          if (col <= r) atomicAdd(p, -c[i][j][2 * h]);
+          if (col + 1 <= r) atomicAdd(p + 1, -c[i][j][2 * h + 1]);
+        }
       }
     }
   }
 }
 
 constexpr int CUD = 68;
-template <int TM>
+enum { CU_ALL = 0, CU_NEXT = 1, CU_REST = 2 };
 __global__ void __launch_bounds__(C_THREADS, 2) chol_update_kernel(int n, int lda, int k0, int t0, int mode,
                                                                     double* __restrict__ A, int band_end, int arrow_lo,
-                                                                    int all_red, int ntiles) {
-  constexpr int WN = TM == 64 ? 4 : 8;
-  constexpr int NJ = 64 / WN / 8;
+                                                                    int all_red) {
   extern __shared__ __align__(16) double cu_smem[];
   double* As = cu_smem;
-  double* Bs = cu_smem + TM * CUD;
-  for (int tile_t = blockIdx.x; tile_t < ntiles; tile_t += gridDim.x) {
+  double* Bs = cu_smem + CT * CUD;
   int bi, bj;
   {
-    int t = tile_t;
-    if (TM == 32) {
-      const int T = (n - t0 + 31) / 32;
-      if (t < T) { bi = t; bj = 0; }
-      else { bi = t - T + 2; bj = 1; }
-    } else if (mode == 4) {
+    const int t = blockIdx.x;
+    if (mode == CU_NEXT) {
       const int T = (max(0, min(band_end, n) - t0) + 63) / 64 + (band_end >= n ? 0 : (n - arrow_lo + 63) / 64);
       if (t < T - 2) { bi = 2 + t; bj = 2; }
       else { bi = 3 + (t - (T - 2)); bj = 3; }
@@ -543,35 +552,35 @@
       while ((bi + 1) * (bi + 2) / 2 <= t) ++bi;
       while (bi * (bi + 1) / 2 > t) --bi;
       bj = t - bi * (bi + 1) / 2;
-      const int skip = mode == 5 ? 4 : (mode >= 2 ? 2 : 0);
+      const int skip = mode == CU_REST ? 4 : 0;
       bi += skip;
       bj += skip;
     }
   }
-  const bool diag = TM == 64 && bi == bj;
+  const bool diag = bi == bj;
   const int tid = threadIdx.x, lane = tid & 31, warp = tid >> 5;
   const int T1v = band_end >= n ? (1 << 30) : (band_end - t0) / 64;
   auto vrow = [&](int v) { return v < T1v ? t0 + v * 64 : arrow_lo + (v - T1v) * 64; };
-  const int ri = TM == 64 ? vrow(bi) : t0 + bi * TM, rj = TM == 64 ? vrow(bj) : t0 + bj * 64;
+  const int ri = vrow(bi), rj = vrow(bj);
   const double* bs = diag ? As : Bs;
-  const int wm = warp / WN, wn = warp % WN;
+  const int wm = warp / 4, wn = warp % 4;
   const int g = lane >> 2, q = lane & 3;
-  double c[4][NJ][2];
-#pragma unroll
-  for (int i = 0; i < 4; ++i)
-#pragma unroll
-    for (int j = 0; j < NJ; ++j) c[i][j][0] = c[i][j][1] = 0.0;
+  double c[2][2][4];
+#pragma unroll
+  for (int i = 0; i < 2; ++i)
+#pragma unroll
+    for (int j = 0; j < 2; ++j) c[i][j][0] = c[i][j][1] = c[i][j][2] = c[i][j][3] = 0.0;
   const double* arow = As + (wm * 32 + g) * CUD + q;
-  const double* brow = bs + (wn * (8 * NJ) + g) * CUD + q;
+  const double* brow = bs + (wn * 16 + g) * CUD + q;
 #pragma unroll 1
   for (int half = 0; half < 2; ++half) {
     if (half) __syncthreads();
-    for (int e = tid; e < (TM + 64) * 16; e += C_THREADS) {
+    for (int e = tid; e < 2 * CT * 16; e += C_THREADS) {
       const int row = e >> 4, ch = (e & 15) * 4;
-      const bool isA = row < TM;
+      const bool isA = row < CT;
       if (!isA && diag) continue;
-      const int grow = isA ? ri + row : rj + (row - TM);
-      double* dst = (isA ? As + row * CUD : Bs + (row - TM) * CUD) + ch;
+      const int grow = isA ? ri + row : rj + (row - CT);
+      double* dst = (isA ? As + row * CUD : Bs + (row - CT) * CUD) + ch;
       if (grow < n) {
         const double* src = A + (size_t)grow * lda + k0 + half * 64 + ch;
         cp_async16(dst, src);
@@ -584,42 +593,49 @@
     cp_async_commit();
     cp_async_wait<0>();
     __syncthreads();
-#pragma unroll 4
-    for (int k4 = 0; k4 < 16; ++k4) {
-      double a[4], b[NJ];
-#pragma unroll
-      for (int i = 0; i < 4; ++i) a[i] = arow[i * 8 * CUD + k4 * 4];
-#pragma unroll
-      for (int j = 0; j < NJ; ++j) b[j] = brow[j * 8 * CUD + k4 * 4];
-#pragma unroll
-      for (int i = 0; i < 4; ++i)
-#pragma unroll
-        for (int j = 0; j < NJ; ++j) chol_dmma(c[i][j][0], c[i][j][1], a[i], b[j]);
-    }
-  }
-#pragma unroll
-  for (int i = 0; i < 4; ++i) {
-    const int r = ri + wm * 32 + i * 8 + g;
-    if (r >= n) continue;
-#pragma unroll
-    for (int j = 0; j < NJ; ++j) {
-      const int col = rj + wn * (8 * NJ) + j * 8 + 2 * q;
-      if (col > r) continue;
-      double* p = A + (size_t)r * lda + col;
-      if (TM == 64 && (all_red || (mode == 3 && bj < 4) || mode == 4 || (mode == 5 && bj < 6))) {
-        atomicAdd(p, -c[i][j][0]);
-        if (col + 1 <= r) atomicAdd(p + 1, -c[i][j][1]);
-      } else if (col + 1 <= r) {
-        double2 v = *reinterpret_cast<double2*>(p);
-        v.x -= c[i][j][0];
-        v.y -= c[i][j][1];
-        *reinterpret_cast<double2*>(p) = v;
-      } else {
-        *p -= c[i][j][0];
-      }
-    }
-  }
-  __syncthreads();
+#pragma unroll 2
+    for (int kk = 0; kk < 64; kk += 16) {
+      double a[2][8], b[2][4];
+#pragma unroll
+      for (int i = 0; i < 2; ++i)
+#pragma unroll
+        for (int e = 0; e < 8; ++e) a[i][e] = arow[(i * 16 + 8 * (e & 1)) * CUD + kk + 4 * (e >> 1)];
+#pragma unroll
+      for (int j = 0; j < 2; ++j)
+#pragma unroll
+        for (int e = 0; e < 4; ++e) b[j][e] = brow[j * 8 * CUD + kk + 4 * e];
+#pragma unroll
+      for (int i = 0; i < 2; ++i)
+#pragma unroll
+        for (int j = 0; j < 2; ++j) dmma_m16n8k16(c[i][j], a[i], b[j]);
+    }
+  }
+  const bool red = all_red || mode == CU_NEXT || (mode == CU_REST && bj < 6);
+#pragma unroll
+  for (int i = 0; i < 2; ++i) {
+#pragma unroll
+    for (int h = 0; h < 2; ++h) {
+      const int r = ri + wm * 32 + i * 16 + g + 8 * h;
+      if (r >= n) continue;
+#pragma unroll
+      for (int j = 0; j < 2; ++j) {
+        const int col = rj + wn * 16 + j * 8 + 2 * q;
+        if (col > r) continue;
+        double* p = A + (size_t)r * lda + col;
+        const double v0 = c[i][j][2 * h], v1 = c[i][j][2 * h + 1];
+        if (red) {
+          atomicAdd(p, -v0);
+          if (col + 1 <= r) atomicAdd(p + 1, -v1);
+        } else if (col + 1 <= r) {
+          double2 v = *reinterpret_cast<double2*>(p);
+          v.x -= v0;
+          v.y -= v1;
+          *reinterpret_cast<double2*>(p) = v;
+        } else {
+          *p -= v0;
+        }
+      }
+    }
   }
 }
 
@@ -632,8 +648,8 @@
 namespace {
 
 struct CholStreams {
-  cudaStream_t side = nullptr, side_lo = nullptr, side_mid = nullptr, cap = nullptr;
-  cudaEvent_t ev_col = nullptr, ev_panel = nullptr, ev_upd[2] = {nullptr, nullptr}, ev_bulk[3] = {nullptr, nullptr, nullptr};
+  cudaStream_t side_lo = nullptr, side_mid = nullptr, cap = nullptr;
+  cudaEvent_t ev_col = nullptr, ev_upd[2] = {nullptr, nullptr}, ev_bulk[3] = {nullptr, nullptr, nullptr};
   bool ready = false;
 };
 
@@ -642,12 +658,10 @@
   if (!s.ready) {
     int lo = 0, hi = 0;
     VGG_CUDA_CHECK(cudaDeviceGetStreamPriorityRange(&lo, &hi));
-    VGG_CUDA_CHECK(cudaStreamCreateWithPriority(&s.side, cudaStreamNonBlocking, hi));
     VGG_CUDA_CHECK(cudaStreamCreateWithPriority(&s.side_lo, cudaStreamNonBlocking, lo));
     VGG_CUDA_CHECK(cudaStreamCreateWithPriority(&s.side_mid, cudaStreamNonBlocking, (lo + hi) / 2));
     VGG_CUDA_CHECK(cudaStreamCreateWithPriority(&s.cap, cudaStreamNonBlocking, hi));
     VGG_CUDA_CHECK(cudaEventCreateWithFlags(&s.ev_col, cudaEventDisableTiming));
-    VGG_CUDA_CHECK(cudaEventCreateWithFlags(&s.ev_panel, cudaEventDisableTiming));
     VGG_CUDA_CHECK(cudaEventCreateWithFlags(&s.ev_upd[0], cudaEventDisableTiming));
     VGG_CUDA_CHECK(cudaEventCreateWithFlags(&s.ev_upd[1], cudaEventDisableTiming));
     for (int i = 0; i < 3; ++i) VGG_CUDA_CHECK(cudaEventCreateWithFlags(&s.ev_bulk[i], cudaEventDisableTiming));
@@ -662,17 +676,25 @@
   return v;
 }
 
+int chol_sms() {
+  static const int v = [] {
+    int dev = 0, sms = 0;
+    if (cudaGetDevice(&dev) != cudaSuccess || cudaDeviceGetAttribute(&sms, cudaDevAttrMultiProcessorCount, dev) != cudaSuccess)
+      sms = 0;
+    return sms > 0 ? sms : 132;
+  }();
+  return v;
+}
+
 int chol_set_attrs() {
   static bool done = false;
   if (done) return VGG_OK;
   VGG_CUDA_CHECK(cudaFuncSetAttribute(chol_panel_kernel<0>, cudaFuncAttributeMaxDynamicSharedMemorySize,
-                                      (int)(sizeof(double) * (CB + C_RPC) * CLD)));
+                                      (int)(sizeof(double) * (CB + C_RPC_MAX) * CLD)));
   VGG_CUDA_CHECK(cudaFuncSetAttribute(chol_panel_kernel<1>, cudaFuncAttributeMaxDynamicSharedMemorySize,
-                                      (int)(sizeof(double) * (CB + C_RPC) * CLD)));
-  VGG_CUDA_CHECK(cudaFuncSetAttribute(chol_update_kernel<64>, cudaFuncAttributeMaxDynamicSharedMemorySize,
+                                      (int)(sizeof(double) * (CB + C_RPC_MAX) * CLD)));
+  VGG_CUDA_CHECK(cudaFuncSetAttribute(chol_update_kernel, cudaFuncAttributeMaxDynamicSharedMemorySize,
                                       (int)(sizeof(double) * 2 * CT * CUD)));
-  VGG_CUDA_CHECK(cudaFuncSetAttribute(chol_update_kernel<32>, cudaFuncAttributeMaxDynamicSharedMemorySize,
-                                      (int)(sizeof(double) * (32 + CT) * CUD)));
   done = true;
   return VGG_OK;
 }
@@ -684,28 +706,20 @@
 
 namespace {
 
-bool chol_fuse() {
-  static const bool v = [] { const char* e = getenv("VGG_CHOL_FUSE"); return !(e && e[0] == '0'); }();
-  return v;
+int chol_panel_rows(int below1, int below2, int* chunks) {
+  const int sms = chol_sms();
+  int xr = C_RPC;
+  for (;; xr += 4) {
+    *chunks = (below1 + xr - 1) / xr + (below2 + xr - 1) / xr;
+    if (1 + *chunks <= sms || xr >= C_RPC_MAX) return xr;
+  }
 }
 
 int chol_enqueue(int n, int lda, double* A, double* Ldiag, int* info, int* flags, cudaStream_t st, CholStreams* cs,
                  bool lookahead) {
   const int nblk = (n + CB - 1) / CB;
-  const size_t smem_p = sizeof(double) * (CB + C_RPC) * CLD;
   const size_t smem_u = sizeof(double) * 2 * CT * CUD;
-  const bool fuse = lookahead && chol_fuse();
-  static const int persist_ctas = [] {
-    const char* e = getenv("VGG_CHOL_PERSIST");
-    if (!(e && e[0] == '1')) return 0;
-    int dev = 0, sms = 132;
-    cudaGetDevice(&dev);
-    cudaDeviceGetAttribute(&sms, cudaDevAttrMultiProcessorCount, dev);
-    return sms;
-  }();
-  auto upd_grid = [&](int tiles) { return persist_ctas > 0 ? std::min(tiles, persist_ctas) : tiles; };
-  static const bool split = [] { const char* e = getenv("VGG_CHOL_SPLIT"); return !(e && e[0] == '0'); }();
-  const bool banded = fuse && split && (int)g_chol_band_end.size() >= nblk && g_chol_arrow_blk > 0;
+  const bool banded = lookahead && (int)g_chol_band_end.size() >= nblk && g_chol_arrow_blk > 0;
   auto band_rows = [&](int b, int* band_end, int* arrow_lo) {
     if (!banded) {
       *band_end = *arrow_lo = n;
@@ -715,94 +729,69 @@
     *arrow_lo = std::min(n, std::max(g_chol_arrow_blk * CB, *band_end));
     if (*band_end >= n || *arrow_lo <= *band_end) *band_end = *arrow_lo = n;
   };
-  auto panel = [&](int b, cudaStream_t s2) -> int {
+  auto panel = [&](int b) -> int {
     const int k0 = b * CB;
-    int band_end, arrow_lo;
+    int band_end, arrow_lo, chunks;
     band_rows(b, &band_end, &arrow_lo);
     const int below1 = std::max(0, std::min(band_end, n) - (k0 + CB));
     const int below2 = band_end >= n ? 0 : n - arrow_lo;
-    const int chunks = (below1 + C_RPC - 1) / C_RPC + (below2 + C_RPC - 1) / C_RPC;
+    const int xr = chol_panel_rows(below1, below2, &chunks);
+    const size_t smem_p = sizeof(double) * (CB + xr) * CLD;
+    const int fuse = lookahead ? 1 : 0;
     if (chol_leaf() == 1)
-      chol_panel_kernel<1><<<1 + chunks, C_THREADS, smem_p, s2>>>(n, lda, k0, A, Ldiag, info, flags, fuse ? 1 : 0, band_end, arrow_lo);
+      chol_panel_kernel<1><<<1 + chunks, C_THREADS, smem_p, st>>>(n, lda, k0, A, Ldiag, info, flags, fuse, band_end, arrow_lo, xr);
     else
-      chol_panel_kernel<0><<<1 + chunks, C_THREADS, smem_p, s2>>>(n, lda, k0, A, Ldiag, info, flags, fuse ? 1 : 0, band_end, arrow_lo);
+      chol_panel_kernel<0><<<1 + chunks, C_THREADS, smem_p, st>>>(n, lda, k0, A, Ldiag, info, flags, fuse, band_end, arrow_lo, xr);
     VGG_LAUNCH_CHECK();
     return VGG_OK;
   };
   int rc;
-  if ((rc = panel(0, st))) return rc;
-  if (fuse) {
-    static const bool skip_bulk = getenv("VGG_CHOL_TIMING_SKIP_BULK") != nullptr;
-    bool have_u1[2] = {false, false}, have_u2[3] = {false, false, false};
+  if ((rc = panel(0))) return rc;
+  if (!lookahead) {
     for (int b = 0; b + 1 < nblk; ++b) {
       const int k0 = b * CB, t0 = k0 + CB;
-      int band_end, arrow_lo;
-      band_rows(b, &band_end, &arrow_lo);
-      const int T = (std::max(0, std::min(band_end, n) - t0) + CT - 1) / CT + (band_end >= n ? 0 : (n - arrow_lo + CT - 1) / CT);
-      const int all_red = band_end >= n ? 0 : 1;
-      const int n_u1 = T > 2 ? (T - 2) + (T > 3 ? T - 3 : 0) : 0;
-      const int n_u2 = T > 4 ? (T - 4) * (T - 3) / 2 : 0;
-      const int n_rest = T > 2 ? (T - 2) * (T - 1) / 2 : 0;
-      have_u1[b & 1] = false;
-      have_u2[b % 3] = false;
-      if (n_rest > 0 && !skip_bulk) {
-        VGG_CUDA_CHECK(cudaEventRecord(cs->ev_col, st));
-        if (split) {
-          VGG_CUDA_CHECK(cudaStreamWaitEvent(cs->side_mid, cs->ev_col, 0));
-          if (b >= 2 && have_u2[(b - 2) % 3]) VGG_CUDA_CHECK(cudaStreamWaitEvent(cs->side_mid, cs->ev_bulk[(b - 2) % 3], 0));
-          chol_update_kernel<64><<<upd_grid(n_u1), C_THREADS, smem_u, cs->side_mid>>>(n, lda, k0, t0, 4, A, band_end, arrow_lo, all_red, n_u1);
-          VGG_LAUNCH_CHECK();
-          VGG_CUDA_CHECK(cudaEventRecord(cs->ev_upd[b & 1], cs->side_mid));
-          have_u1[b & 1] = true;
-          if (n_u2 > 0) {
-            VGG_CUDA_CHECK(cudaStreamWaitEvent(cs->side_lo, cs->ev_col, 0));
-            chol_update_kernel<64><<<upd_grid(n_u2), C_THREADS, smem_u, cs->side_lo>>>(n, lda, k0, t0, 5, A, band_end, arrow_lo, all_red, n_u2);
-            VGG_LAUNCH_CHECK();
-            VGG_CUDA_CHECK(cudaEventRecord(cs->ev_bulk[b % 3], cs->side_lo));
-            have_u2[b % 3] = true;
-          }
-        } else {
-          VGG_CUDA_CHECK(cudaStreamWaitEvent(cs->side_lo, cs->ev_col, 0));
-          chol_update_kernel<64><<<upd_grid(n_rest), C_THREADS, smem_u, cs->side_lo>>>(n, lda, k0, t0, 3, A, n, n, 0, n_rest);
-          VGG_LAUNCH_CHECK();
-          VGG_CUDA_CHECK(cudaEventRecord(cs->ev_upd[b & 1], cs->side_lo));
-          have_u1[b & 1] = true;
-        }
-      }
-      if (b >= 1 && have_u1[(b - 1) & 1]) VGG_CUDA_CHECK(cudaStreamWaitEvent(st, cs->ev_upd[(b - 1) & 1], 0));
-      if (b >= 2 && have_u2[(b - 2) % 3]) VGG_CUDA_CHECK(cudaStreamWaitEvent(st, cs->ev_bulk[(b - 2) % 3], 0));
-      if ((rc = panel(b + 1, st))) return rc;
-    }
-    for (int i = 0; i < 2; ++i)
-      if (have_u1[i]) VGG_CUDA_CHECK(cudaStreamWaitEvent(st, cs->ev_upd[i], 0));
-    for (int i = 0; i < 3; ++i)
-      if (have_u2[i]) VGG_CUDA_CHECK(cudaStreamWaitEvent(st, cs->ev_bulk[i], 0));
+      const int T = (n - t0 + CT - 1) / CT;
+      chol_update_kernel<<<T * (T + 1) / 2, C_THREADS, smem_u, st>>>(n, lda, k0, t0, CU_ALL, A, n, n, 0);
+      VGG_LAUNCH_CHECK();
+      if ((rc = panel(b + 1))) return rc;
+    }
     return VGG_OK;
   }
+  bool have_u1[2] = {false, false}, have_u2[3] = {false, false, false};
   for (int b = 0; b + 1 < nblk; ++b) {
     const int k0 = b * CB, t0 = k0 + CB;
-    const int T = (n - t0 + CT - 1) / CT;
-    const int T32 = (n - t0 + 31) / 32;
-    const int n_col = T32 + (T32 > 2 ? T32 - 2 : 0);
-    const int n_rest = T > 2 ? (T - 2) * (T - 1) / 2 : 0;
-    if (!lookahead) {
-      chol_update_kernel<64><<<upd_grid(T * (T + 1) / 2), C_THREADS, smem_u, st>>>(n, lda, k0, t0, 0, A, n, n, 0, T * (T + 1) / 2);
+    int band_end, arrow_lo;
+    band_rows(b, &band_end, &arrow_lo);
+    const int T = (std::max(0, std::min(band_end, n) - t0) + CT - 1) / CT + (band_end >= n ? 0 : (n - arrow_lo + CT - 1) / CT);
+    const int all_red = band_end >= n ? 0 : 1;
+    const int n_u1 = T > 2 ? (T - 2) + (T > 3 ? T - 3 : 0) : 0;
+    const int n_u2 = T > 4 ? (T - 4) * (T - 3) / 2 : 0;
+    have_u1[b & 1] = false;
+    have_u2[b % 3] = false;
+    if (n_u1 > 0) {
+      VGG_CUDA_CHECK(cudaEventRecord(cs->ev_col, st));
+      VGG_CUDA_CHECK(cudaStreamWaitEvent(cs->side_mid, cs->ev_col, 0));
+      if (b >= 2 && have_u2[(b - 2) % 3]) VGG_CUDA_CHECK(cudaStreamWaitEvent(cs->side_mid, cs->ev_bulk[(b - 2) % 3], 0));
+      chol_update_kernel<<<n_u1, C_THREADS, smem_u, cs->side_mid>>>(n, lda, k0, t0, CU_NEXT, A, band_end, arrow_lo, all_red);
       VGG_LAUNCH_CHECK();
-      if ((rc = panel(b + 1, st))) return rc;
-      continue;
-    }
-    chol_update_kernel<32><<<n_col, C_THREADS, sizeof(double) * (32 + CT) * CUD, st>>>(n, lda, k0, t0, 1, A, n, n, 0, n_col);
-    VGG_LAUNCH_CHECK();
-    VGG_CUDA_CHECK(cudaEventRecord(cs->ev_col, st));
-    VGG_CUDA_CHECK(cudaStreamWaitEvent(cs->side, cs->ev_col, 0));
-    if ((rc = panel(b + 1, cs->side))) return rc;
-    VGG_CUDA_CHECK(cudaEventRecord(cs->ev_panel, cs->side));
-    if (n_rest > 0) {
-      chol_update_kernel<64><<<upd_grid(n_rest), C_THREADS, smem_u, st>>>(n, lda, k0, t0, 2, A, n, n, 0, n_rest);
-      VGG_LAUNCH_CHECK();
-    }
-    VGG_CUDA_CHECK(cudaStreamWaitEvent(st, cs->ev_panel, 0));
-  }
+      VGG_CUDA_CHECK(cudaEventRecord(cs->ev_upd[b & 1], cs->side_mid));
+      have_u1[b & 1] = true;
+      if (n_u2 > 0) {
+        VGG_CUDA_CHECK(cudaStreamWaitEvent(cs->side_lo, cs->ev_col, 0));
+        chol_update_kernel<<<n_u2, C_THREADS, smem_u, cs->side_lo>>>(n, lda, k0, t0, CU_REST, A, band_end, arrow_lo, all_red);
+        VGG_LAUNCH_CHECK();
+        VGG_CUDA_CHECK(cudaEventRecord(cs->ev_bulk[b % 3], cs->side_lo));
+        have_u2[b % 3] = true;
+      }
+    }
+    if (b >= 1 && have_u1[(b - 1) & 1]) VGG_CUDA_CHECK(cudaStreamWaitEvent(st, cs->ev_upd[(b - 1) & 1], 0));
+    if (b >= 2 && have_u2[(b - 2) % 3]) VGG_CUDA_CHECK(cudaStreamWaitEvent(st, cs->ev_bulk[(b - 2) % 3], 0));
+    if ((rc = panel(b + 1))) return rc;
+  }
+  for (int i = 0; i < 2; ++i)
+    if (have_u1[i]) VGG_CUDA_CHECK(cudaStreamWaitEvent(st, cs->ev_upd[i], 0));
+  for (int i = 0; i < 3; ++i)
+    if (have_u2[i]) VGG_CUDA_CHECK(cudaStreamWaitEvent(st, cs->ev_bulk[i], 0));
   return VGG_OK;
 }
 
diff --git a/vggsfm_b200/csrc/common.cuh b/vggsfm_b200/csrc/common.cuh
--- a/vggsfm_b200/csrc/common.cuh
+++ b/vggsfm_b200/csrc/common.cuh
@@ -133,6 +133,15 @@
   asm volatile("cp.async.wait_group %0;" ::"n"(N) : "memory");
 }
 
+__device__ __forceinline__ void dmma_m16n8k16(double (&d)[4], const double (&a)[8], const double (&b)[4]) {
+  asm volatile(
+      "mma.sync.aligned.m16n8k16.row.col.f64.f64.f64.f64 {%0,%1,%2,%3}, {%4,%5,%6,%7,%8,%9,%10,%11}, {%12,%13,%14,%15}, "
+      "{%0,%1,%2,%3};"
+      : "+d"(d[0]), "+d"(d[1]), "+d"(d[2]), "+d"(d[3])
+      : "d"(a[0]), "d"(a[1]), "d"(a[2]), "d"(a[3]), "d"(a[4]), "d"(a[5]), "d"(a[6]), "d"(a[7]), "d"(b[0]), "d"(b[1]),
+        "d"(b[2]), "d"(b[3]));
+}
+
 template <int KP>
 __device__ __forceinline__ double warp_reduce_scatter(double (&v)[KP], int lane) {
 #pragma unroll
```

Measured after the change: 295.3, median of 6. 3.5% higher.
